# weleen/AGRL.pytorch

Hardware: AMD Instinct MI355X
Metric: frames/sec (fwd+GCN+distmat), MARS seq_len=8 (higher is better)
Workload: dtype fp16; 1 GPU; MARS seq_len=8 bs=32/GPU fp16 fwd+distmat (BASELINE configs[1]): 256x128 frames, VMGN ResNet50x2-branch + 2 graph layers, cosine distmat vs resident 12180 x 4096 gallery; global_batch=32, seq_len=8, gallery_rows_per_gpu=12180, parallelism=dp1, hip_graph=False, ranks=1, devices_visible=1, library=libagrl_hip.so, clip_batches_rotated=3, clip_bytes_rotated=301989888

## Files before the change

### agrl.pytorch_amd/csrc/agrl_common.h

```cpp
#pragma once
#include <hip/hip_runtime.h>
#include <math.h>
#include <stdint.h>
#include <stdio.h>
#include <stdarg.h>

#include "../../include/agrl_hip.h"

#define AGRL_WAVE 64

#ifndef AGRL_LP_F16
#define AGRL_LP_F16 1
#endif
constexpr bool kLpF16 = AGRL_LP_F16 != 0;
typedef unsigned short lp16_t;
typedef __attribute__((ext_vector_type(8))) __bf16 bf16x8_t;
typedef __attribute__((ext_vector_type(8))) _Float16 f16x8_t;
typedef __attribute__((ext_vector_type(4))) float f32x4_t;

void agrl_set_error(const char* fmt, ...);

#define AGRL_CHECK_ARG(cond, ...)       \
    do {                                \
        if (!(cond)) {                  \
            agrl_set_error(__VA_ARGS__); \
            return 1;                   \
        }                               \
    } while (0)

#define AGRL_CHECK_LAUNCH(name)                                                   \
    do {                                                                          \
        hipError_t e__ = hipGetLastError();                                       \
        if (e__ != hipSuccess) {                                                  \
            agrl_set_error("%s: launch failed: %s", name, hipGetErrorString(e__)); \
            return 2;                                                             \
        }                                                                         \
    } while (0)

static inline bool agrl_is_pow2(float v) {
    int e = 0;
    return v > 0.f && v <= 3.4e38f && frexpf(v, &e) == 0.5f;
}
#define AGRL_CHECK_POW2(value, who, name) \
    AGRL_CHECK_ARG(agrl_is_pow2(value), "%s: %s=%g is not a positive finite power of two", who, name, (double)(value))

__attribute__((visibility("hidden"))) int agrl_cu_count();

typedef __attribute__((address_space(3))) void lds_void_t;
typedef __attribute__((address_space(1))) const void gbl_void_t;

__host__ __device__ inline float lp16_to_f32(lp16_t v) {
    if constexpr (kLpF16) {
        return (float)__builtin_bit_cast(_Float16, v);
    } else {
        return __builtin_bit_cast(float, ((uint32_t)v) << 16);
    }
}

__host__ __device__ inline lp16_t f32_to_lp16(float f) {
    if constexpr (kLpF16) {
        return __builtin_bit_cast(unsigned short, (_Float16)f);
    } else {
#if defined(__HIP_DEVICE_COMPILE__)
        const __bf16 h = (__bf16)f;
        return __builtin_bit_cast(unsigned short, h);
#else
        uint32_t u = __builtin_bit_cast(uint32_t, f);
        if ((u & 0x7fffffffu) > 0x7f800000u) return (lp16_t)((u >> 16) | 0x40);
        u += 0x7fffu + ((u >> 16) & 1u);
        return (lp16_t)(u >> 16);
#endif
    }
}

__device__ inline uint32_t pack_lp16x2(float lo, float hi) {
    if constexpr (kLpF16) {
        typedef __attribute__((ext_vector_type(2))) _Float16 f16x2_t;
        const f16x2_t v = {(_Float16)lo, (_Float16)hi};
        return __builtin_bit_cast(uint32_t, v);
    } else {
        typedef __attribute__((ext_vector_type(2))) __bf16 bf16x2_t;
        const bf16x2_t v = {(__bf16)lo, (__bf16)hi};
        return __builtin_bit_cast(uint32_t, v);
    }
}

__device__ inline uint32_t pack_bf16x2(float lo, float hi) {
    typedef __attribute__((ext_vector_type(2))) __bf16 bf16x2_t;
    const bf16x2_t v = {(__bf16)lo, (__bf16)hi};
    return __builtin_bit_cast(uint32_t, v);
}

__device__ inline void unpack_lp16x2(uint32_t w, float& lo, float& hi) {
    if constexpr (kLpF16) {
        typedef __attribute__((ext_vector_type(2))) _Float16 f16x2_t;
        const f16x2_t v = __builtin_bit_cast(f16x2_t, w);
        lo = (float)v[0];
        hi = (float)v[1];
    } else {
        lo = __uint_as_float(w << 16);
        hi = __uint_as_float(w & 0xffff0000u);
    }
}

template <typename TA, typename TB>
__device__ inline __attribute__((ext_vector_type(4))) float mfma_lp16_16x16x32(const TA& a, const TB& b, __attribute__((ext_vector_type(4))) float c) {
    static_assert(sizeof(TA) == 16 && sizeof(TB) == 16, "16-byte MFMA operands");
    if constexpr (kLpF16) {
        return __builtin_amdgcn_mfma_f32_16x16x32_f16(__builtin_bit_cast(f16x8_t, a), __builtin_bit_cast(f16x8_t, b), c, 0, 0, 0);
    } else {
        return __builtin_amdgcn_mfma_f32_16x16x32_bf16(__builtin_bit_cast(bf16x8_t, a), __builtin_bit_cast(bf16x8_t, b), c, 0, 0, 0);
    }
}

__device__ inline float relu_nan(float v) { return __builtin_elementwise_maximum(v, 0.f); }

__device__ inline float wave_sum(float v) {
#pragma unroll
    for (int off = 32; off > 0; off >>= 1) v += __shfl_xor(v, off, 64);
    return v;
}

__device__ inline float wave_max(float v) {
#pragma unroll
    for (int off = 32; off > 0; off >>= 1) v = fmaxf(v, __shfl_xor(v, off, 64));
    return v;
}

__device__ inline int wave_sum_i(int v) {
#pragma unroll
    for (int off = 32; off > 0; off >>= 1) v += __shfl_xor(v, off, 64);
    return v;
}

template <typename T>
struct DT;
template <>
struct DT<float> {
    static constexpr int code = AGRL_F32;
    static constexpr int epc = 4;
    __device__ static inline float ld(const float* p) { return *p; }
    __device__ static inline void st(float* p, float v) { *p = v; }
};
struct f32s_t {
    float v;
};
template <>
struct DT<f32s_t> {
    static constexpr int code = AGRL_F32X3;
    static constexpr int epc = 4;
};
struct f32h_t {
    float v;
};
template <>
struct DT<f32h_t> {
    static constexpr int code = AGRL_F32H3;
    static constexpr int epc = 4;
};
template <>
struct DT<lp16_t> {
    static constexpr int code = AGRL_LP16;
    static constexpr int epc = 8;
    __device__ static inline float ld(const lp16_t* p) { return lp16_to_f32(*p); }
    __device__ static inline void st(lp16_t* p, float v) { *p = f32_to_lp16(v); }
};

static inline int cdiv(int a, int b) { return (a + b - 1) / b; }

#define AGRL_OPT_UNSET (-2147483647 - 1)
struct AgrlOpts {
    int igemm_wide;
    int pool_persist;
    int conv3x3_wide, conv3x3_c64;
    int distmat_tiled;
    int topk_radix;
    int graph_linear_mmajor;
    int conv3x3_n128;
    int conv3x3_fat_pb;
    int conv3x3_half, conv3x3_half_stagger;
    int stem_split_lds;
    int stem_xcd_map;
    int stem_regpool;
    int distmat_tile_n;
    int split16_ns;
    int duo_persist;
    int igemm_dbg, conv3x3_dbg;
};
const AgrlOpts& agrl_opts();
inline bool agrl_opt_set(int v) { return v != AGRL_OPT_UNSET; }

#ifdef AGRL_ABLATE
#define AGRL_DBG_BITS(p) ((p).dbg)
#else
#define AGRL_DBG_BITS(p) 0
#endif
```

### agrl.pytorch_amd/csrc/bottleneck_seam.hip

```cpp
#include <utility>

#include "igemm_dev.h"

namespace {

struct SeamParams {
    const unsigned char* y2;
    const unsigned char* wpk;
    const float* b3;
    const unsigned char* res;
    unsigned char* out;
    const float* b1n;
    unsigned char* z;
    int M;
};

#ifndef SEAM_ABL
#define SEAM_ABL 0
#endif
constexpr int SBM = 128;
constexpr int SCH = 256;

template <typename F, int... Is>
__device__ __forceinline__ void static_for_impl(F&& f, std::integer_sequence<int, Is...>) {
    (f(std::integral_constant<int, Is>{}), ...);
}
template <int N, typename F>
__device__ __forceinline__ void static_for(F&& f) {
    static_for_impl(f, std::make_integer_sequence<int, N>{});
}

typedef unsigned u32x4_t __attribute__((ext_vector_type(4)));
typedef __attribute__((address_space(3))) unsigned char lds_u8_t;
typedef __attribute__((address_space(3))) u32x4_t lds_u32x4_t;
__device__ __forceinline__ u32x4_t lds_ld16(const lds_u8_t* p) {
#if SEAM_ABL & 16
    return u32x4_t{(unsigned)(size_t)p, 1u, 2u, 3u};
#else
    return *reinterpret_cast<const lds_u32x4_t*>(p);
#endif
}

template <int IMM>
__device__ __forceinline__ void gload16_asm(u32x4_t& dst, unsigned off, const unsigned char* base) {
    static_assert(IMM >= 0 && IMM < 4096, "13-bit signed immediate");
    asm volatile("global_load_dwordx4 %0, %1, %2 offset:%3" : "=v"(dst) : "v"(off), "s"(base), "n"(IMM) : "memory");
}
template <int RQ>
__device__ __forceinline__ void mfma_v(f32x4_t& acc, const u32x4_t& b) {
    if constexpr (kLpF16) asm volatile("v_mfma_f32_16x16x32_f16 %0, a[%c2:%c3], %1, %0" : "+v"(acc) : "v"(b), "n"(4 * RQ), "n"(4 * RQ + 3));
    else asm volatile("v_mfma_f32_16x16x32_bf16 %0, a[%c2:%c3], %1, %0" : "+v"(acc) : "v"(b), "n"(4 * RQ), "n"(4 * RQ + 3));
}
template <int AQ, int RQ>
__device__ __forceinline__ void mfma_a(const u32x4_t& b) {
    if constexpr (kLpF16)
        asm volatile("v_mfma_f32_16x16x32_f16 a[%c1:%c2], a[%c3:%c4], %0, a[%c1:%c2]" ::"v"(b), "n"(4 * AQ), "n"(4 * AQ + 3), "n"(4 * RQ), "n"(4 * RQ + 3));
    else
        asm volatile("v_mfma_f32_16x16x32_bf16 a[%c1:%c2], a[%c3:%c4], %0, a[%c1:%c2]" ::"v"(b), "n"(4 * AQ), "n"(4 * AQ + 3), "n"(4 * RQ), "n"(4 * RQ + 3));
}
template <int AQ>
__device__ __forceinline__ void acc_zero() {
    asm volatile("v_accvgpr_write_b32 a[%c0], 0\n\tv_accvgpr_write_b32 a[%c1], 0\n\tv_accvgpr_write_b32 a[%c2], 0\n\tv_accvgpr_write_b32 a[%c3], 0" ::"n"(4 * AQ),
                 "n"(4 * AQ + 1), "n"(4 * AQ + 2), "n"(4 * AQ + 3));
}
template <int AQ>
__device__ __forceinline__ f32x4_t acc_read() {
    float x, y, z, w;
    asm volatile("v_accvgpr_read_b32 %0, a[%c4]\n\tv_accvgpr_read_b32 %1, a[%c5]\n\tv_accvgpr_read_b32 %2, a[%c6]\n\tv_accvgpr_read_b32 %3, a[%c7]"
                 : "=v"(x), "=v"(y), "=v"(z), "=v"(w)
                 : "n"(4 * AQ), "n"(4 * AQ + 1), "n"(4 * AQ + 2), "n"(4 * AQ + 3));
    return f32x4_t{x, y, z, w};
}
template <int IMM>
__device__ __forceinline__ void gstore16_asm(const u32x4_t& v, unsigned off, unsigned char* base) {
    asm volatile("global_store_dwordx4 %0, %1, %2 offset:%3\n\ts_nop 1" ::"v"(off), "v"(v), "s"(base), "n"(IMM) : "memory");
}
template <int RQ, int IMM>
__device__ __forceinline__ void ring_load(unsigned off, const unsigned char* base) {
    static_assert(IMM >= 0 && IMM < 4096, "13-bit signed immediate");
    asm volatile("global_load_dwordx4 a[%c2:%c3], %0, %1 offset:%4" ::"v"(off), "s"(base), "n"(4 * RQ), "n"(4 * RQ + 3), "n"(IMM) : "memory");
}
__device__ __forceinline__ void mfma_drain() { asm volatile("s_nop 15\n\ts_nop 15" ::: "memory"); }

__device__ __forceinline__ void dma16s(const unsigned char* sbase, unsigned voff, unsigned lds_wave_addr) {
    unsigned keep;
    asm volatile(
        "s_mov_b32 %0, m0\n\ts_mov_b32 m0, %3\n\ts_nop 0\n\tglobal_load_lds_dwordx4 %1, %2\n\ts_mov_b32 m0, %0"
        : "=&s"(keep)
        : "v"(voff), "s"(sbase), "s"(lds_wave_addr)
        : "memory");
}

constexpr int NWV = 4;
constexpr int FW1 = 4;
constexpr int Y2P = 4;
constexpr int S_OPS = (SEAM_ABL & 1) ? 0 : 32;
template <int KS1, int FW2, bool Y2RING, int RING>
struct Sched {
    static constexpr int G1F = FW1 * KS1, G2F = 8 * FW2, FPC = G1F + G2F;
    int allowed[FPC];
};
template <int KS1, int FW2, bool Y2RING, int RING>
constexpr Sched<KS1, FW2, Y2RING, RING> make_sched() {
    using S = Sched<KS1, FW2, Y2RING, RING>;
    S s{};
    int issued[4][S::FPC] = {};
    int seq = 0;
    for (int p = 0; p < RING; ++p) issued[0][p] = seq++;
    for (int k = 0; k < 3; ++k) {
        for (int p = 0; p < S::FPC; ++p) {
            if (p == S::G1F) seq += S_OPS;
            if (k == 1) s.allowed[p] = seq - 1 - issued[k][p];
            if (Y2RING && p < S::G1F && (p % FW1) == FW1 - 1 && ((p / FW1) & 1)) seq += Y2P;
            const int q = p + RING;
            if (q >= S::FPC) issued[k + 1][q - S::FPC] = seq++;
            else issued[k][q] = seq++;
        }
    }
    return s;
}
template <int KS1, int FW2, bool Y2RING, int RING>
struct SchedOf {
    static constexpr Sched<KS1, FW2, Y2RING, RING> value = make_sched<KS1, FW2, Y2RING, RING>();
};

template <int K1, int N1, int N2>
__global__ __launch_bounds__(NWV * 64) void bottleneck_seam_kernel(const SeamParams p) {
    static_assert((K1 == 256 || K1 == 512) && N1 % SCH == 0 && (N2 == 256 || N2 == 512), "shapes");
    constexpr int NC = N1 / SCH;
    constexpr int KS1 = K1 / 32;
    constexpr int FW2 = N2 / 64;
    constexpr bool Y2RING = K1 > 256;
    constexpr int NKT = K1 / 64;
    constexpr int NSL = 5, AHEAD = 3;
    constexpr int XO = Y2RING ? NSL * 16384 : 64 * 1024;
    constexpr int BIAS_OFF = XO + 64 * 1024;
    constexpr int RING = N2 == 256 ? 16 : 8;
    constexpr int NA2 = (64 - RING) < FW2 * 8 ? (64 - RING) : FW2 * 8;
    constexpr int NV2 = FW2 * 8 - NA2;
    using SCHED = SchedOf<KS1, FW2, Y2RING, RING>;
    constexpr int G1F = FW1 * KS1, G2F = 8 * FW2, FPC = G1F + G2F;
    static_assert(FPC % RING == 0, "the ring index of a fragment must not depend on the chunk");

    __shared__ __attribute__((aligned(16))) unsigned char smem_[BIAS_OFF + N1 * 4];
    lds_u8_t* const smem = (lds_u8_t*)smem_;
    const unsigned lds0 = (unsigned)(size_t)smem;

    const int tid = threadIdx.x;
    const int lane = tid & 63;
    const int wave = __builtin_amdgcn_readfirstlane(tid >> 6);
    const int frow = lane & 15, fchunk = lane >> 4;
    const int m0 = blockIdx.x * SBM;
    const unsigned lane16 = (unsigned)lane * 16u;

    unsigned a_off[2];
#pragma unroll
    for (int j = 0; j < 2; ++j) {
        const int row = wave * 32 + j * 8 + (lane >> 3);
        a_off[j] = (unsigned)(m0 + row) * (K1 * 2) + (unsigned)(((lane & 7) ^ ((row >> 1) & 7)) << 4);
    }
    const unsigned ldsA = __builtin_amdgcn_readfirstlane(lds0 + wave * 4096);
    auto issue_y2 = [&](int kt, int slot) {
        const unsigned char* src = p.y2 + kt * 128;
        const unsigned dst = ldsA + slot * 16384;
        dma16s(src, a_off[0], dst);
        dma16s(src, a_off[1], dst + 1024);
        dma16s(src + 16 * (K1 * 2), a_off[0], dst + 2048);
        dma16s(src + 16 * (K1 * 2), a_off[1], dst + 3072);
    };
    const int lo128 = frow * 128 + ((fchunk ^ ((frow >> 1) & 7)) << 4);
    const unsigned r_off = (unsigned)(m0 + frow) * (N1 * 2) + (unsigned)(wave * 64 + 8 * fchunk) * 2;

    const lds_u8_t* xptr = smem + XO + lane16;
    const lds_u8_t* sa0 = smem + lo128;
    const lds_u8_t* sa1 = smem + (lo128 ^ 64);
    asm volatile("" : "+v"(xptr), "+v"(sa0), "+v"(sa1));

    auto issue_w = [&](auto slot_c, const unsigned char* chunk_base, auto pos_c) {
        constexpr int SLOT = decltype(slot_c)::value, POS = decltype(pos_c)::value;
        if constexpr (SEAM_ABL & 8) return;
        ring_load<SLOT, (POS & 3) * 1024>(lane16, chunk_base + (POS & ~3) * 1024);
    };
    auto chunk_stream = [&](int c) { return p.wpk + (size_t)(c * NWV + wave) * (FPC * 1024); };

    f32x4_t acc1[FW1][8];
    asm volatile("" ::: "a255");
    static_for<NA2>([&](auto qc) { acc_zero<RING + decltype(qc)::value>(); });
    f32x4_t acc2v[NV2 > 0 ? NV2 : 1];
#pragma unroll
    for (int i = 0; i < (NV2 > 0 ? NV2 : 1); ++i) acc2v[i] = f32x4_t{0.f, 0.f, 0.f, 0.f};

    u32x4_t rres[8][2];
    auto load_residual = [&](int c) {
        const unsigned char* rc = p.res + (size_t)c * (SCH * 2);
#pragma unroll
        for (int b = 0; b < 8; ++b) {
            if constexpr (SEAM_ABL & 1) { rres[b][0] = u32x4_t{(unsigned)c, r_off, 1u, 2u}; rres[b][1] = rres[b][0]; continue; }
            gload16_asm<0>(rres[b][0], r_off, rc + b * (16 * N1 * 2));
            gload16_asm<64>(rres[b][1], r_off, rc + b * (16 * N1 * 2));
        }
    };
    auto init_acc1 = [&](int c) {
#pragma unroll
        for (int j = 0; j < 2; ++j) {
            float bias[8];
            {
                const lds_u8_t* bs = smem + BIAS_OFF + (c * SCH + wave * 64 + 32 * j + 8 * fchunk) * 4;
                const u32x4_t b0 = *reinterpret_cast<const lds_u32x4_t*>(bs), b1 = *reinterpret_cast<const lds_u32x4_t*>(bs + 16);
#pragma unroll
                for (int e = 0; e < 4; ++e) { bias[e] = __uint_as_float(b0[e]); bias[4 + e] = __uint_as_float(b1[e]); }
            }
#pragma unroll
            for (int b = 0; b < 8; ++b) {
                const uint32_t w4[4] = {rres[b][j][0], rres[b][j][1], rres[b][j][2], rres[b][j][3]};
                float v[8];
#pragma unroll
                for (int e = 0; e < 4; ++e) unpack_lp16x2(w4[e], v[2 * e], v[2 * e + 1]);
#pragma unroll
                for (int e = 0; e < 8; ++e) v[e] = (SEAM_ABL & 1) ? bias[e] : v[e] + bias[e];
                acc1[2 * j][b] = f32x4_t{v[0], v[1], v[2], v[3]};
                acc1[2 * j + 1][b] = f32x4_t{v[4], v[5], v[6], v[7]};
                __builtin_amdgcn_sched_barrier(0);
            }
        }
    };

    using std::integral_constant;

    load_residual(0);
#pragma unroll
    for (int i = 0; i < N1 / 1024; ++i)
        dma16s(reinterpret_cast<const unsigned char*>(p.b3) + (wave * (N1 / 1024) + i) * 1024, lane16, lds0 + BIAS_OFF + (wave * (N1 / 1024) + i) * 1024);
#pragma unroll
    for (int t = 0; t < (Y2RING ? AHEAD : NKT); ++t) issue_y2(t, t);
    {
        const unsigned char* s0 = chunk_stream(0);
        static_for<RING>([&](auto ic) { issue_w(ic, s0, ic); });
    }
    asm volatile("s_waitcnt vmcnt(%0)" ::"n"((SEAM_ABL & 8) ? 0 : RING) : "memory");
    __builtin_amdgcn_s_barrier();
    asm volatile("" ::: "memory");

    u32x4_t bf[8];
    int kt_slot = 0;
    int slot_off = 0;
    auto ld_y2 = [&](auto ks_c, int b) {
        constexpr int KS = decltype(ks_c)::value;
        const lds_u8_t* base = (KS & 1) ? sa1 : sa0;
        if constexpr (Y2RING) return lds_ld16(base + slot_off + b * 2048);
        else return lds_ld16(base + (KS >> 1) * 16384 + b * 2048);
    };

    for (int c = 0;; ++c) {
        const bool last = c + 1 == NC;
        const int cn = last ? 0 : c + 1;
        const unsigned char* ws = chunk_stream(c);
        const unsigned char* wsn = chunk_stream(cn);

#pragma unroll
        for (int b = 0; b < 8; ++b) asm volatile("" : "+v"(rres[b][0]), "+v"(rres[b][1]));
        init_acc1(c);
        __builtin_amdgcn_sched_barrier(0);
#pragma unroll
        for (int b = 0; b < 8; ++b) bf[b] = ld_y2(integral_constant<int, 0>{}, b);
        asm volatile("s_nop 4" ::: "memory");

        static_for<FPC>([&](auto pc) {
            constexpr int P = decltype(pc)::value;
            constexpr bool G1 = P < G1F;
            constexpr int F = G1 ? P : P - G1F;
            constexpr int FW = G1 ? FW1 : FW2;
            constexpr int KS = F / FW, A = F % FW;
            constexpr int SL = P % RING;
            constexpr bool LAST_A = A + 1 == FW;

            if constexpr (P == G1F) {
                if constexpr (!Y2RING) {
                    __builtin_amdgcn_s_barrier();
                    asm volatile("" ::: "memory");
                }
                mfma_drain();
                unsigned char* oc = p.out + (size_t)c * (SCH * 2);
                const lds_u8_t* xw = xptr + wave * 16384;
                static_for<2>([&](auto jc) {
                    constexpr int j = decltype(jc)::value;
#pragma unroll
                    for (int b = 0; b < 8; ++b) {
                        float v[8];
#pragma unroll
                        for (int e = 0; e < 4; ++e) {
                            v[e] = relu_nan(acc1[2 * j][b][e]);
                            v[4 + e] = relu_nan(acc1[2 * j + 1][b][e]);
                        }
                        const u32x4_t pk = {pack_lp16x2(v[0], v[1]), pack_lp16x2(v[2], v[3]), pack_lp16x2(v[4], v[5]), pack_lp16x2(v[6], v[7])};
                        if constexpr (!(SEAM_ABL & 1)) gstore16_asm<j * 64>(pk, r_off, oc + b * (16 * N1 * 2));
                        *reinterpret_cast<lds_u32x4_t*>(const_cast<lds_u8_t*>(xw) + (j * 8 + b) * 1024) = pk;
                    }
                });
                load_residual(cn);
                wg_barrier();
#pragma unroll
                for (int b = 0; b < 8; ++b) bf[b] = lds_ld16(xptr + b * 1024);
            }

            if constexpr (!(SEAM_ABL & 8)) wait_vmcnt<SCHED::value.allowed[P]>();

            if constexpr (Y2RING && G1 && LAST_A && (KS & 1)) {
                __builtin_amdgcn_s_barrier();
                asm volatile("" ::: "memory");
                const int nslot = (kt_slot + (KS >> 1) + 1) % NSL;
                issue_y2(((KS >> 1) + AHEAD) % NKT, (nslot + AHEAD - 1) % NSL);
                slot_off = nslot * 16384;
            }
            static_for<8>([&](auto bc) {
                constexpr int b = decltype(bc)::value;
                if constexpr (G1) {
                    if constexpr (SEAM_ABL & 2) asm volatile("" ::"v"(bf[b]));
                    else mfma_v<SL>(acc1[A][b], bf[b]);
                } else {
                    if constexpr (SEAM_ABL & 4) asm volatile("" ::"v"(bf[b]));
                    else if constexpr (A * 8 + b < NA2) mfma_a<RING + A * 8 + b, SL>(bf[b]);
                    else mfma_v<SL>(acc2v[A * 8 + b - NA2], bf[b]);
                }
                if constexpr (LAST_A) {
                    if constexpr (G1 && KS + 1 < KS1) {
                        __builtin_amdgcn_sched_barrier(0);
                        bf[b] = ld_y2(integral_constant<int, KS + 1>{}, b);
                    } else if constexpr (!G1 && KS + 1 < 8) {
                        __builtin_amdgcn_sched_barrier(0);
                        bf[b] = lds_ld16(xptr + ((KS + 1) * 8 + b) * 1024);
                    }
                }
            });
            __builtin_amdgcn_sched_barrier(0);
            constexpr int Q = P + RING;
            if constexpr (Q >= FPC) issue_w(integral_constant<int, SL>{}, wsn, integral_constant<int, Q - FPC>{});
            else issue_w(integral_constant<int, SL>{}, ws, integral_constant<int, Q>{});
            if constexpr (Y2RING && P + 1 == G1F) kt_slot = (kt_slot + NKT) % NSL;
        });
        if (last) break;
    }
    asm volatile("s_waitcnt vmcnt(0)" ::: "memory");
    mfma_drain();

    unsigned lane_z;
    asm volatile("v_mbcnt_lo_u32_b32 %0, -1, 0\n\tv_mbcnt_hi_u32_b32 %0, -1, %0" : "=v"(lane_z));
    const int frow_z = lane_z & 15, fchunk_z = lane_z >> 4;
    lp16_t* __restrict__ zp = reinterpret_cast<lp16_t*>(p.z);
    const int cb2 = wave * (N2 / NWV) + 8 * fchunk_z;
    static_for<FW2 / 2>([&](auto jc) {
        constexpr int j = decltype(jc)::value;
        const float4 b0 = *reinterpret_cast<const float4*>(p.b1n + cb2 + 32 * j);
        const float4 b1 = *reinterpret_cast<const float4*>(p.b1n + cb2 + 32 * j + 4);
        static_for<8>([&](auto bc) {
            constexpr int b = decltype(bc)::value;
            const int gm = m0 + b * 16 + frow_z;
            f32x4_t lo, hi;
            if constexpr ((2 * j) * 8 + b < NA2) lo = acc_read<RING + (2 * j) * 8 + b>();
            else lo = acc2v[(2 * j) * 8 + b - NA2];
            if constexpr ((2 * j + 1) * 8 + b < NA2) hi = acc_read<RING + (2 * j + 1) * 8 + b>();
            else hi = acc2v[(2 * j + 1) * 8 + b - NA2];
            float v[8];
            v[0] = lo[0] + b0.x; v[1] = lo[1] + b0.y; v[2] = lo[2] + b0.z; v[3] = lo[3] + b0.w;
            v[4] = hi[0] + b1.x; v[5] = hi[1] + b1.y; v[6] = hi[2] + b1.z; v[7] = hi[3] + b1.w;
#pragma unroll
            for (int e = 0; e < 8; ++e) v[e] = relu_nan(v[e]);
            *reinterpret_cast<uint4*>(zp + (size_t)gm * N2 + cb2 + 32 * j) =
                make_uint4(pack_lp16x2(v[0], v[1]), pack_lp16x2(v[2], v[3]), pack_lp16x2(v[4], v[5]), pack_lp16x2(v[6], v[7]));
        });
    });
}

__global__ void seam_pack_kernel(const lp16_t* __restrict__ w3, const lp16_t* __restrict__ w1n, uint4* __restrict__ wpk, int K1, int N1, int N2) {
    const int KS1 = K1 / 32, FW2 = N2 / 64, G1F = FW1 * KS1, FPC = G1F + 8 * FW2;
    const long long total = (long long)(N1 / SCH) * NWV * FPC * 64;
    for (long long t = blockIdx.x * (long long)blockDim.x + threadIdx.x; t < total; t += (long long)gridDim.x * blockDim.x) {
        const int lane = (int)(t & 63);
        long long r = t >> 6;
        const int q = (int)(r % FPC);
        r /= FPC;
        const int w = (int)(r % NWV), c = (int)(r / NWV);
        const int i = lane & 15, f = lane >> 4;
        const lp16_t* src;
        if (q < G1F) {
            const int ks = q / FW1, a = q % FW1;
            const int ch = c * SCH + w * 64 + 32 * (a >> 1) + 8 * (i >> 2) + 4 * (a & 1) + (i & 3);
            src = w3 + (size_t)ch * K1 + ks * 32 + f * 8;
        } else {
            const int g = q - G1F, ks = g / FW2, a = g % FW2;
            const int och = w * (N2 / NWV) + 32 * (a >> 1) + 8 * (i >> 2) + 4 * (a & 1) + (i & 3);
            src = w1n + (size_t)och * N1 + c * SCH + ks * 32 + f * 8;
        }
        wpk[t] = *reinterpret_cast<const uint4*>(src);
    }
}

bool seam_shape_ok(int Cmid, int Cout, int Cnext) {
    return (Cmid == 256 && Cout == 1024 && Cnext == 256) || (Cmid == 512 && Cout == 2048 && Cnext == 512) ||
           (Cmid == 256 && Cout == 1024 && Cnext == 512);
}

}

extern "C" long long agrl_bottleneck_seam_packed_bytes(int Cmid, int Cout, int Cnext) {
    if (!seam_shape_ok(Cmid, Cout, Cnext)) return 0;
    return ((long long)Cout * Cmid + (long long)Cnext * Cout) * 2;
}

extern "C" int agrl_bottleneck_seam_pack(const void* w3, const void* w1_next, void* packed, int Cmid, int Cout, int Cnext,
                                         agrl_stream_t stream) {
    AGRL_CHECK_ARG(w3 && w1_next && packed, "agrl_bottleneck_seam_pack: null pointer");
    AGRL_CHECK_ARG(seam_shape_ok(Cmid, Cout, Cnext), "agrl_bottleneck_seam_pack: built for 256/1024/256, 256/1024/512 and 512/2048/512 channels, got %d/%d/%d",
                   Cmid, Cout, Cnext);
    AGRL_CHECK_ARG((((uintptr_t)w3 | (uintptr_t)w1_next | (uintptr_t)packed) & 15) == 0, "agrl_bottleneck_seam_pack: pointers must be 16-byte aligned");
    hipLaunchKernelGGL(seam_pack_kernel, dim3(512), dim3(256), 0, (hipStream_t)stream, reinterpret_cast<const lp16_t*>(w3),
                       reinterpret_cast<const lp16_t*>(w1_next), reinterpret_cast<uint4*>(packed), Cmid, Cout, Cnext);
    AGRL_CHECK_LAUNCH("agrl_bottleneck_seam_pack");
    return 0;
}

extern "C" int agrl_bottleneck_seam(const void* y2, const void* packed, const float* b3, const void* residual, void* out,
                                    const float* b1_next, void* z, int M, int Cmid, int Cout, int Cnext, agrl_stream_t stream) {
    AGRL_CHECK_ARG(y2 && packed && b3 && residual && out && b1_next && z, "agrl_bottleneck_seam: null pointer");
    AGRL_CHECK_ARG(seam_shape_ok(Cmid, Cout, Cnext), "agrl_bottleneck_seam: built for 256/1024/256, 256/1024/512 and 512/2048/512 channels, got %d/%d/%d",
                   Cmid, Cout, Cnext);
    AGRL_CHECK_ARG(M > 0 && M % SBM == 0, "agrl_bottleneck_seam: the pixel count must be a multiple of %d (whole 16 x 8 frames), got %d", SBM, M);
    AGRL_CHECK_ARG((size_t)M * Cout * 2 < (1ull << 32), "agrl_bottleneck_seam: maps beyond 4 GB are not addressed");
    const uintptr_t al = (uintptr_t)y2 | (uintptr_t)packed | (uintptr_t)b3 | (uintptr_t)residual | (uintptr_t)out | (uintptr_t)b1_next | (uintptr_t)z;
    AGRL_CHECK_ARG((al & 15) == 0, "agrl_bottleneck_seam: pointers must be 16-byte aligned");
    SeamParams p;
    p.y2 = reinterpret_cast<const unsigned char*>(y2);
    p.wpk = reinterpret_cast<const unsigned char*>(packed);
    p.b3 = b3;
    p.res = reinterpret_cast<const unsigned char*>(residual);
    p.out = reinterpret_cast<unsigned char*>(out);
    p.b1n = b1_next;
    p.z = reinterpret_cast<unsigned char*>(z);
    p.M = M;
    const dim3 grid(M / SBM), block(NWV * 64);
    if (Cmid == 256 && Cnext == 256) hipLaunchKernelGGL((bottleneck_seam_kernel<256, 1024, 256>), grid, block, 0, (hipStream_t)stream, p);
    else if (Cmid == 256) hipLaunchKernelGGL((bottleneck_seam_kernel<256, 1024, 512>), grid, block, 0, (hipStream_t)stream, p);
    else hipLaunchKernelGGL((bottleneck_seam_kernel<512, 2048, 512>), grid, block, 0, (hipStream_t)stream, p);
    AGRL_CHECK_LAUNCH("agrl_bottleneck_seam");
    return 0;
}
```

### agrl.pytorch_amd/csrc/common.hip

```cpp
#include "agrl_common.h"

static thread_local char g_err[512] = "";

void agrl_set_error(const char* fmt, ...) {
    va_list ap;
    va_start(ap, fmt);
    vsnprintf(g_err, sizeof(g_err), fmt, ap);
    va_end(ap);
}

extern "C" int agrl_version(void) { return 100; }
extern "C" const char* agrl_last_error(void) { return g_err; }

extern "C" int agrl_lp16_is_f16(void) { return kLpF16 ? 1 : 0; }

#include <atomic>

int agrl_cu_count() {
    constexpr int kMaxDev = 64;
    static std::atomic<int> cache[kMaxDev];
    int dev = 0;
    if (hipGetDevice(&dev) != hipSuccess) return 256;
    const bool slot = dev >= 0 && dev < kMaxDev;
    int n = slot ? cache[dev].load(std::memory_order_relaxed) : 0;
    if (n > 0) return n;
    if (hipDeviceGetAttribute(&n, hipDeviceAttributeMultiprocessorCount, dev) != hipSuccess || n <= 0) n = 256;
    if (slot) cache[dev].store(n, std::memory_order_relaxed);
    return n;
}

#include <stdlib.h>

static int opt_int(const char* name) {
    const char* e = getenv(name);
    return e ? atoi(e) : AGRL_OPT_UNSET;
}
static int opt_flag(const char* name) {
    const char* e = getenv(name);
    return e && !(e[0] == '0' && e[1] == 0) ? 1 : 0;
}
static AgrlOpts load_opts() {
    AgrlOpts o;
    o.igemm_wide = opt_int("AGRL_IGEMM_WIDE");
    o.pool_persist = opt_flag("AGRL_POOL_PERSIST");
    o.conv3x3_wide = opt_int("AGRL_CONV3X3_WIDE");
    o.conv3x3_c64 = opt_int("AGRL_CONV3X3_C64");
    o.distmat_tiled = opt_flag("AGRL_DISTMAT_TILED");
    o.topk_radix = opt_flag("AGRL_TOPK_RADIX");
    o.graph_linear_mmajor = opt_flag("AGRL_GRAPH_LINEAR_MMAJOR");
    o.conv3x3_n128 = opt_flag("AGRL_CONV3X3_N128");
    o.distmat_tile_n = opt_int("AGRL_DISTMAT_TILE_N");
    o.duo_persist = opt_int("AGRL_DUO_PERSIST");
    o.split16_ns = opt_int("AGRL_SPLIT16_NS");
    o.stem_xcd_map = opt_int("AGRL_STEM_XCD_MAP");
    o.stem_split_lds = opt_int("AGRL_STEM_SPLIT_LDS");
    o.stem_regpool = opt_int("AGRL_STEM_REGPOOL");
    o.conv3x3_fat_pb = opt_int("AGRL_CONV3X3_FAT_PB");
    o.conv3x3_half = opt_int("AGRL_CONV3X3_HALF");
    o.conv3x3_half_stagger = opt_int("AGRL_CONV3X3_HALF_STAGGER");
#ifdef AGRL_ABLATE
    o.igemm_dbg = agrl_opt_set(opt_int("AGRL_IGEMM_DBG")) ? opt_int("AGRL_IGEMM_DBG") : 0;
    o.conv3x3_dbg = agrl_opt_set(opt_int("AGRL_CONV3X3_DBG")) ? opt_int("AGRL_CONV3X3_DBG") : 0;
#else
    o.igemm_dbg = 0;
    o.conv3x3_dbg = 0;
#endif
    return o;
}
static AgrlOpts g_opts = load_opts();

const AgrlOpts& agrl_opts() { return g_opts; }
extern "C" int agrl_reload_options(void) {
    g_opts = load_opts();
    return 0;
}
extern "C" int agrl_built_with_ablation(void) {
#ifdef AGRL_ABLATE
    return 1;
#else
    return 0;
#endif
}
```

### agrl.pytorch_amd/torchreid/_hip.py

```python
from __future__ import annotations

import ctypes as C
import os
import threading

import torch

F32 = 0
LP16 = 1
F32X3 = 2
F32H3P = 4
F32H3 = 3
FRAMES_NCHW = 0
FRAMES_NHWC = 1
METRIC_EUCLIDEAN = 0
METRIC_COSINE = 1

LP_NAME = os.environ.get("AGRL_HIP_LP16")
if LP_NAME is None:
    LP_NAME = os.environ.get("AGRL_HIP_PRECISION") if os.environ.get("AGRL_HIP_PRECISION") in ("fp16", "bf16") else "fp16"
if LP_NAME not in ("fp16", "bf16"):
    raise ValueError("AGRL_HIP_LP16 must be fp16 or bf16, not %r" % LP_NAME)
LP_DTYPE = torch.float16 if LP_NAME == "fp16" else torch.bfloat16

_HERE = os.path.dirname(os.path.abspath(__file__))
LIB_PATH = os.environ.get(
    "AGRL_HIP_LIB", os.path.normpath(os.path.join(_HERE, "..", "lib", "libagrl_hip.so" if LP_NAME == "fp16" else "libagrl_hip_bf16.so"))
)


class HipLibraryError(RuntimeError):
    """libagrl_hip.so is missing or incomplete."""


class HipKernelError(RuntimeError):
    """An entry point of libagrl_hip.so returned a non-zero status."""


_p = C.c_void_p
_i = C.c_int
_f = C.c_float

SIGNATURES = {
    "agrl_stem_conv_bn_relu_maxpool": [_p, _p, _p, _p, _i, _i, _i, _i, _p],
    "agrl_stem_conv_bn_relu_maxpool_lp16": [_p, _p, _p, _p, _i, _i, _i, _p],
    "agrl_conv2d_bn_act": [_p, _p, _p, _p, _p, _i, _i, _i, _i, _i, _i, _i, _i, _i, _i, _i, _p],
    "agrl_conv1x1_dual_split16": [_p, _p, _p, _p, _p] + [_i] * 8 + [_f, _i, _i, _p],
    "agrl_stem_split16": [_p, _p, _p, _p, _p, _i, _i, _i, _f, _p],
    "agrl_stem_conv_bn_relu_maxpool_u8": [_p, _p, _i, _p, _p, _p, _i, _i, _i, _i, _p],
    "agrl_stem_conv_bn_relu_maxpool_lp16_u8": [_p, _p, _i, _p, _p, _p, _i, _i, _i, _p],
    "agrl_stem_split16_u8": [_p, _p, _i, _p, _p, _p, _p, _i, _i, _i, _f, _p],
    "agrl_frames_normalize_u8": [_p, _p, _i, _p, _i, _i, _i, _p],
    "agrl_clip_resample_u8": [_p, _p, _p, _i, _i, _i, _i, _i, _p],
    "agrl_resample_taps_u8": [_i, _i, _p, _p, _p],
    "agrl_split16_planes": [_p, _p, C.c_longlong, _i, _i, _p],
    "agrl_split16_weight_planes": [_p, _p, C.c_longlong, _i, _f, _p],
    "agrl_split16_weights_inloop": [_p, _p, C.c_longlong, _i, _p],
    "agrl_conv1x1_split16": [_p, _p, _p, _p, _p, _i, _i, _i, _i, _f, _i, _p],
    "agrl_conv1x1_split16_dual": [_p, _p, _p, _p, _p, _i, _i, _i, _i, _i, _f, _i, _p],
    "agrl_conv1x1_split16_pool": [_p, _p, _p, _p, _p, _i, _i, _i, _i, _i, _i, C.POINTER(_i), _i, _i, _f, _i, _p],
    "agrl_conv3x3_packed_split16": [_p, _p, _p, _p, _i, _i, _i, _i, _i, _i, _f, _p],
    "agrl_conv2d_bn_act_split16": [_p, _p, _p, _p, _p] + [_i] * 10 + [_f, _i, _i, _p],
    "agrl_bottleneck_tail": [_p, _p, _p, _p, _p, _p, _p, _p, _p, _p, _p, _i, _i, _i, _i, _i, _p],
    "agrl_bottleneck_seam_packed_bytes": [_i, _i, _i],
    "agrl_bottleneck_seam_pack": [_p, _p, _p, _i, _i, _i, _p],
    "agrl_bottleneck_seam": [_p, _p, _p, _p, _p, _p, _p, _i, _i, _i, _i, _p],
    "agrl_conv3x3_packed_bytes": [_i, _i],
    "agrl_conv1x1_packed_bytes": [_i, _i],
    "agrl_conv1x1_pack": [_p, _p, _i, _i, _p],
    "agrl_conv1x1_packed_bn_act": [_p, _p, _p, _p, _p, _i, _i, _i, _i, _i, _p],
    "agrl_conv1x1_packed_res_bn_act": [_p, _p, _p, _p, _p, _i, _i, _i, _i, _p],
    "agrl_conv1x1_packed_res_pool": [_p, _p, _p, _p, _p, _p, _i, _i, _i, _i, _i, _i, C.POINTER(_i), _i, _i, _p],
    "agrl_conv1x1_packed_dual_duo": [_p, _p, _p, _p, _p, _i, _i, _i, _i, _i, _p],
    "agrl_conv1x1_packed_dual_strided": [_p, _p, _p, _p, _p, _i, _i, _i, _i, _i, _i, _i, _i, _p],
    "agrl_conv3x3_pack": [_p, _p, _i, _i, _p],
    "agrl_conv3x3_packed_bn_act": [_p, _p, _p, _p, _i, _i, _i, _i, _i, _i, _p],
    "agrl_bottleneck_block": [_p, _p, _p, _p, _p, _p, _p, _p, _p, _p, _p, _p, _p, _i, _i, _i, _i, _i, _i, _p],
    "agrl_conv1x1_dual_bn_act": [_p, _p, _p, _p, _p, _i, _i, _i, _i, _i, _p],
    "agrl_conv1x1_bn_act_pool": [_p, _p, _p, _p, _p, _p, _p, _i, _i, _i, _i, _i, _i, C.POINTER(_i), _i, _i, _p],
    "agrl_linear_nobias": [_p, _p, _p, _i, _i, _i, _i, _p],
    "agrl_part_pool": [_p, _p, _p, _p, _p, _i, _i, _i, _i, C.POINTER(_i), _i, _i, _p],
    "agrl_clip_pool": [_p, _p, _i, _i, _i, _i, _p],
    "agrl_clip_pool_ragged": [_p, _p, _p, _p, _i, _i, _i, _i, _p],
    "agrl_graph_gram": [_p, _p, _i, _i, _i, _i, _p],
    "agrl_graph_pair_product": [_p, _p, _p, _p, _i, _i, _i, _p],
    "agrl_graph_finalize": [_p, _i, _p, _p, _i, _i, _i, _i, _i, _p],
    "agrl_graph_propagate": [_p, _p, _p, _p, _p, _f, _f, _f, _p, _p, _i, _i, _i, _p],
    "agrl_pam_pool": [_p, _p, _p, _p, _i, _i, _i, _i, _i, C.POINTER(_i), _i, _i, _p],
    "agrl_pam_combine": [_p, _p, _p, _f, _p, _p, _i, _i, _p],
    "agrl_pam_pool_train": [_p, _p, _p, _p, _p, _i, _i, _i, _i, _i, C.POINTER(_i), _i, _i, _p],
    "agrl_pam_pool_backward": [_p, _p, _p, _p, _p, _p, _p, _i, _i, _i, _i, _i, C.POINTER(_i), _i, _i, _p],
    "agrl_pam_combine_train": [_p, _p, _p, _p, _p, _i, _i, _p],
    "agrl_pam_combine_backward": [_p, _p, _p, _p, _p, _p, _p, _p, _i, _i, _p, C.c_size_t, _p],
    "agrl_col_sum_workspace": [_i, _i],
    "agrl_col_sum": [_p, _p, _i, _i, _p, C.c_size_t, _p],
    "agrl_graph_apply": [_p, _p, _p, _i, _i, _i, _i, _p],
    "agrl_graph_tracklet_operand": [_p, _p, _i, _p, _p, _i, _i, _i, _i, _i, _i, _i, _p],
    "agrl_graph_finalize_bits": [_p, _i, _p, _p, _i, _i, _i, _i, _i, _p],
    "agrl_pose_adjacency_bits": [_p, _p, _p, _i, _i, _i, _i, C.c_float, C.c_float, _p],
    "agrl_adjacency_pack": [_p, _p, _i, _i, _p],
    "agrl_graph_linear_mix": [_p, _p, _p, _p, _p, _f, _f, _f, _p, _i, _i, _i, _i, _p],
    "agrl_row_sqnorm": [_p, _p, _i, _i, _i, _p],
    "agrl_attn_pool_bnneck": [_p, _p, _p, _p, _p, _p, _p, _p, _p, _p, _i, _i, _i, _i, _i, _p],
    "agrl_sta_frame_stats": [_p, _p, _p, _p, _i, _i, _i, _i, _i, _p],
    "agrl_sta_fuse": [_p, _p, _p, _p, _p, _p, _i, _i, _i, _i, _i, _i, _p],
    "agrl_linear_bn_relu": [_p, _p, _p, _p, _p, _i, _i, _i, _i, _p],
    "agrl_attn_tail": [_p, _p, _p, _p, _p, _p, _p, _p, _p, _p, _p, _p, _p, _i, _i, _i, _i, _i, _p],
    "agrl_row_l2_normalize": [_p, _p, _i, _i, _i, _i, _i, _p],
    "agrl_distmat_split16": [_p, _p, _p, _p, _p, _i, _i, _i, _i, _i, _f, _p, C.c_size_t, _p],
    "agrl_distmat": [_p, _p, _p, _p, _p, _i, _i, _i, _i, _i, _i, _p, C.c_size_t, _p],
    "agrl_pose_adjacency": [_p, _p, _p, _i, _i, _i, _i, C.c_float, C.c_float, _p],
    "agrl_re_ranking_workspace": [_i, _i, _i],
    "agrl_re_ranking": [_p, _p, _p, _i, _i, _i, _i, C.c_double, _p, _i, _p, C.c_size_t, _p],
    "agrl_rank_topk": [_p, _i, _i, _i, _i, _i, _p, _p, _p],
    "agrl_distmat_topk_workspace": [_i, _i],
    "agrl_distmat_topk": [_p, _p, _p, _p, _i, _i, _i, _i, _i, _i, _i, _p, _p, _p, C.c_size_t, _p, C.c_size_t, _p],
    "agrl_rank_argsort": [_p, _i, _i, _i, _p, _p],
    "agrl_rank_mars": [_p, _p, _p, _p, _p, _i, _i, _i, _p, _p, _p],
    "agrl_rank_market1501": [_p, _i, _i, _i, _p, _p, _p, _p, _i, _p, _p, _p, _p],
    "agrl_triplet_hard_mine": [_p, _p, _i, _i, _p, _p, _p, _p, _p],
    "agrl_axpby": [_p, _p, _f, _f, _p, C.c_size_t, _p],
    "agrl_part_pool_backward": [_p, _p, _p, _p, _i, _i, _i, _i, _i, C.POINTER(_i), _i, _p],
    "agrl_attn_pool_backward": [_p, _p, _p, _i, _i, _i, _i, _p],
    "agrl_graph_matrix_backward": [_p, _i, _p, _p, _i, _i, _i, _i, _p],
    "agrl_xent_label_smooth": [_p, _p, _i, _i, _f, _p, _p, _p, _p],
    "agrl_triplet_loss": [_p, _p, _i, _i, _f, _i, _p, _p, _p, _p, _p, _p, _p, _p],
    "agrl_bn_workspace": [_i, _i],
    "agrl_bn_stats": [_p, _p, _p, _i, _i, _p, C.c_size_t, _p],
    "agrl_conv2d_stats": [_p, _p, _p, _p, C.c_size_t] + [_i] * 10 + [_p],
    "agrl_bn_stats_from_partials": [_p, _i, _i, _i, _p, _p, _p, C.c_size_t, _p],
    "agrl_bn_fold_train": [_p, _p, _p, _p, _f, _f, C.c_longlong, _p, _p, _p, _p, _p, _p, _i, _p],
    "agrl_bn_apply": [_p, _p, _p, _p, _p, _p, _i, _i, _i, _f, _p],
    "agrl_bn_backward": [_p, _p, _p, _p, _p, _p, _p, _i, _f, _p, _p, _p, _p, _i, _i, _p, C.c_size_t, _p],
    "agrl_im2col_t": [_p, _p, _i, _i, _i, _i, _i, _i, _i, _i, _i, _p],
    "agrl_gemm_nt_splitk": [_p, _p, _p, _i, _i, _i, _i, _p, C.c_size_t, _p],
    "agrl_im2col_rows": [_p, _p] + [_i] * 10 + [_p],
    "agrl_conv_wgrad_workspace": [_i] * 9,
    "agrl_conv_wgrad_plan": [_i] * 10 + [C.POINTER(_i)],
    "agrl_conv_wgrad": [_p, _p, _p] + [_i] * 10 + [_p, C.c_size_t, _p],
    "agrl_maxpool3x3s2": [_p, _p, _p, _i, _i, _i, _i, _p],
    "agrl_maxpool3x3s2_backward": [_p, _p, _p, _i, _i, _i, _i, _p],
    "agrl_diag_read_stream": [_p, C.c_size_t, _p, _i, _p],
    "agrl_optim_geometry": [C.POINTER(_i), C.POINTER(_i), C.POINTER(_i)],
    "agrl_adam_step": [_p, _i, _p, _i] + [_f] * 7 + [_i, _i, _p],
    "agrl_sgd_step": [_p, _i, _p, _i, _f, _f, _f, _i, _i, _i, _i, _p],
    "agrl_rmsprop_step": [_p, _i, _p, _i] + [_f] * 6 + [_i, _i, _p],
    "agrl_adabound_step": [_p, _i, _p, _i] + [_f] * 8 + [_i, _i, _p],
    "agrl_radam_step": [_p, _i, _p, _i] + [_f] * 6 + [_i, _i, _p],
}

_lock = threading.Lock()
_lib = None


def lib():
    global _lib
    if _lib is not None:
        return _lib
    with _lock:
        if _lib is not None:
            return _lib
        if not os.path.exists(LIB_PATH):
            raise HipLibraryError(
                "libagrl_hip.so not found at %s -- build it with `python __graft_entry__.py` "
                "(or `make -C agrl.pytorch_amd/csrc`); the HIP path has no fallback" % LIB_PATH
            )
        try:
            h = C.CDLL(LIB_PATH)
        except OSError as e:
            raise HipLibraryError("cannot load %s: %s" % (LIB_PATH, e))
        for name, argtypes in SIGNATURES.items():
            try:
                fn = getattr(h, name)
            except AttributeError:
                raise HipLibraryError("%s does not export %s" % (LIB_PATH, name))
            fn.argtypes = argtypes
            fn.restype = _i
        h.agrl_re_ranking_workspace.restype = C.c_size_t
        h.agrl_bn_workspace.restype = C.c_size_t
        h.agrl_col_sum_workspace.restype = C.c_size_t
        h.agrl_conv_wgrad_workspace.restype = C.c_size_t
        h.agrl_distmat_topk_workspace.restype = C.c_size_t
        h.agrl_bottleneck_seam_packed_bytes.restype = C.c_longlong
        h.agrl_conv3x3_packed_bytes.restype = C.c_longlong
        h.agrl_conv1x1_packed_bytes.restype = C.c_longlong
        for name in ("agrl_reload_options", "agrl_built_with_ablation", "agrl_lp16_is_f16"):
            getattr(h, name).argtypes = []
            getattr(h, name).restype = _i
        h.agrl_version.restype = _i
        h.agrl_last_error.restype = C.c_char_p
        if bool(h.agrl_lp16_is_f16()) != (LP_NAME == "fp16"):
            raise HipLibraryError("%s stores 16-bit data as %s but AGRL_HIP_LP16 asks for %s" % (
                LIB_PATH, "fp16" if h.agrl_lp16_is_f16() else "bf16", LP_NAME))
        _lib = h
    return _lib


RELOAD_HOOKS = []


def reload_options():
    lib().agrl_reload_options()
    for hook in RELOAD_HOOKS:
        hook()


def available() -> bool:
    try:
        lib()
        return True
    except HipLibraryError:
        return False


def _check(name, status):
    if status != 0:
        msg = lib().agrl_last_error()
        raise HipKernelError("%s failed (%d): %s" % (name, status, msg.decode() if msg else "?"))


def stream_ptr(device=None):
    return torch.cuda.current_stream(device).cuda_stream


def ptr(t):
    if t is None:
        return None
    assert t.is_cuda, "HIP entry points take device tensors"
    assert t.is_contiguous(), "HIP entry points take contiguous tensors"
    return t.data_ptr()


def dtype_code(dt):
    if dt == torch.float32:
        return F32
    if dt == LP_DTYPE:
        return LP16
    raise TypeError("unsupported dtype %s (float32 / %s only: the loaded library's 16-bit type is %s)" % (dt, LP_DTYPE, LP_NAME))


PROFILE = None
PROFILE_TAG = None


def call(name, *args):
    fn = getattr(lib(), name)
    if PROFILE is None:
        _check(name, fn(*args))
        return
    stream = torch.cuda.ExternalStream(args[-1]) if args[-1] else torch.cuda.current_stream()
    start, end = torch.cuda.Event(enable_timing=True), torch.cuda.Event(enable_timing=True)
    start.record(stream)
    _check(name, fn(*args))
    end.record(stream)
    global PROFILE_TAG
    PROFILE.append((name, start, end, PROFILE_TAG))
    PROFILE_TAG = None
```

### agrl.pytorch_amd/torchreid/hip_ops.py

```python
from __future__ import annotations

import ctypes as C
import functools
import os

import numpy as np
import torch

from . import _hip
from ._hip import F32, LP16, LP_DTYPE, LP_NAME, METRIC_COSINE, METRIC_EUCLIDEAN, call, dtype_code, ptr


import contextlib
import threading
import weakref

_MODE = threading.local()


@contextlib.contextmanager
def f32_split(on=True):
    prev = getattr(_MODE, 'split', False)
    _MODE.split = bool(on)
    try:
# ... 312 lines not shown
                 _stream(x_nchw))
    return out


def conv_bn_act(x, w_ohwi, bias, stride, pad, relu, residual=None, x_presplit=False, out_presplit=False):
    N, H, W, Cin = x.shape
    Cout, R, S, Cin2 = w_ohwi.shape
    assert Cin == Cin2 and x.dtype == w_ohwi.dtype
    OH, OW = (H + 2 * pad - R) // stride + 1, (W + 2 * pad - S) // stride + 1
    out = torch.empty((N, OH, OW, Cout), dtype=x.dtype, device=x.device)
    if residual is not None:
        assert residual.shape == out.shape and residual.dtype == out.dtype
    if _hip.PROFILE is not None:
        e = x.element_size()
        _hip.PROFILE_TAG = {"flops": 2.0 * N * OH * OW * Cout * R * S * Cin,
                            "bytes": e * (x.numel() + w_ohwi.numel() + out.numel() * (2 if residual is not None else 1)),
                            "conv": (R, stride, Cin, Cout, OH, OW)}
    unscale = getattr(w_ohwi, 'agrl_unscale', None)
    with _dev(x):
        if unscale is not None:
            assert x.dtype == torch.float32 and getattr(w_ohwi, 'agrl_presplit', False), "fp16x3 weights come from split16_inloop_weights"
            call("agrl_conv2d_bn_act_split16", ptr(x), ptr(w_ohwi), ptr(bias), ptr(residual), ptr(out), N, H, W, Cin, Cout, R, S,
                 stride, pad, 1 if relu else 0, float(unscale), 1 if x_presplit else 0, 1 if out_presplit else 0, _stream(x))
        else:
            assert not (x_presplit or out_presplit), "pre-split activations exist in the 'fp16x3' arithmetic only"
            call("agrl_conv2d_bn_act", ptr(x), ptr(w_ohwi), ptr(bias), ptr(residual), ptr(out), N, H, W, Cin, Cout, R, S,
                 stride, pad, 1 if relu else 0, _gemm_code(x.dtype), _stream(x))
    return out


def conv1x1_dual_split16(x, x2, w_cat, bias, stride, relu=True, x2_presplit=False, out_planes=0):
    N, H, W, K1 = x.shape
    K2 = x2.shape[3]
    Cout = w_cat.shape[0]
    OH, OW = (H - 1) // stride + 1, (W - 1) // stride + 1
    assert x.dtype == torch.float32 and x2.dtype == torch.float32 and x.is_contiguous() and x2.is_contiguous()
    assert tuple(x2.shape[:3]) == (N, OH, OW) and tuple(w_cat.shape) == (Cout, K1 + K2) and getattr(w_cat, 'agrl_presplit', False)
    assert out_planes in (0, 2, 3)
    out = (torch.empty((N, OH, OW, out_planes * Cout), dtype=torch.float16, device=x.device) if out_planes
           else torch.empty((N, OH, OW, Cout), dtype=torch.float32, device=x.device))
    if _hip.PROFILE is not None:
        M = N * OH * OW
        _hip.PROFILE_TAG = {"flops": 2.0 * M * Cout * (K1 + K2), "bytes": 4.0 * (M * (K1 + K2) + w_cat.numel()) + out.numel() * out.element_size(),
                            "conv": (1, stride, K1 + K2, Cout, OH, OW)}
    with _dev(x):
        call("agrl_conv1x1_dual_split16", ptr(x), ptr(x2), ptr(w_cat), ptr(bias), ptr(out), N, H, W, stride, K1, K2, Cout,
             1 if relu else 0, float(w_cat.agrl_unscale), 1 if x2_presplit else 0, int(out_planes), _stream(x))
    return out


def split16_prescale(w):
    import math
    amax = float(w.detach().abs().max())
    if not (amax > 0.0 and math.isfinite(amax)):
        k = 0
    else:
        k = 13 - math.frexp(amax)[1] + 1
    ws = (w.detach().float() * (2.0 ** k)).contiguous()
    ws.agrl_unscale = 2.0 ** (-k)
    return ws


def split16_inloop_weights(w):
    ws = split16_prescale(w)
    K = ws.shape[-1]
    assert K % 32 == 0, "the in-loop split needs whole 32-element k-tiles (K = %d)" % K
    t = ws.view(-1, K // 32, 2, 4, 4).permute(0, 1, 3, 2, 4)
    hi = t.to(torch.float16)
    lo = (t - hi.float()).to(torch.float16)
    out = torch.stack([hi, lo], dim=2).contiguous().view(torch.float32).view(ws.shape)
    out.agrl_unscale = ws.agrl_unscale
    out.agrl_presplit = True
    out.agrl_scaled = ws
    return out


def split16_true_weights(t):
    src = t.agrl_scaled if getattr(t, 'agrl_presplit', False) else t
    return src * t.agrl_unscale


def pack_stem_weights_split16(w_ohwi):
    assert tuple(w_ohwi.shape) == (64, 7, 7, 3)
    ws = split16_prescale(w_ohwi)
    w4 = torch.zeros((64, 7, 8, 4), dtype=torch.float32, device=w_ohwi.device)
    w4[:, :, :7, :3] = ws
    wh = w4.to(torch.float16)
    wl = (w4 - wh.float()).to(torch.float16)
    out = []
    for t in (wh, wl):
        packed = torch.zeros((64, 240), dtype=torch.float16, device=w_ohwi.device)
        packed[:, :224] = t.view(64, 224)
        out.append(packed.contiguous())
    return out[0], out[1], ws.agrl_unscale


def stem_split16(x_nchw, wh_packed, wl_packed, unscale, bias, mean=PIXEL_MEAN, std=PIXEL_STD):
    x_nchw, N, H, W, ebytes, u8 = _stem_frames(x_nchw, mean, std)
    CH, CW, PH, PW = stem_out_shape(H, W)
    out = torch.empty((N, PH, PW, 64), dtype=torch.float32, device=x_nchw.device)
    if _hip.PROFILE is not None:
        _hip.PROFILE_TAG = {"flops": 2.0 * N * CH * CW * 64 * 147, "bytes": ebytes * x_nchw.numel() + 4.0 * out.numel() + 4.0 * wh_packed.numel(),
                            "conv": (7, 2, 3, 64, PH, PW)}
    with _dev(x_nchw):
        if u8 is not None:
            call("agrl_stem_split16_u8", ptr(x_nchw), ptr(u8[0]), u8[1], ptr(wh_packed), ptr(wl_packed), ptr(bias), ptr(out), N, H, W,
                 float(unscale), _stream(x_nchw))
        else:
            call("agrl_stem_split16", ptr(x_nchw), ptr(wh_packed), ptr(wl_packed), ptr(bias), ptr(out), N, H, W, float(unscale), _stream(x_nchw))
    return out


def split16_planes_available():
    return LP_NAME == 'fp16'


def split16_plane_weights(w, segments=None, pair_first=False):
    ws = split16_prescale(w)
    parts = []
    for i, seg in enumerate(torch.split(ws, segments or [ws.shape[-1]], dim=-1)):
        wh = seg.to(torch.float16)
        wl = (seg - wh.float()).to(torch.float16)
        wh_s = (wh.float() * (2.0 ** -11)).to(torch.float16)
        if pair_first and i == 0:
            assert seg.shape[-1] % 128 == 0
            lead = tuple(seg.shape[:-1])
            slabs = [t.reshape(lead + (-1, 128)) for t in (wh, wl, wh_s)]
            parts.append(torch.stack(slabs, dim=-2).reshape(lead + (3 * seg.shape[-1],)))
        else:
            parts += [wh, wh_s, wl]
    return torch.cat(parts, dim=-1).contiguous(), ws.agrl_unscale


def to_split16_planes(x, nplanes=3):
    assert x.dtype == torch.float32 and x.is_contiguous() and x.shape[-1] % 4 == 0 and nplanes in (2, 3)
    Cc = x.shape[-1]
    out = torch.empty(tuple(x.shape[:-1]) + (nplanes * Cc,), dtype=torch.float16, device=x.device)
    with _dev(x):
        call("agrl_split16_planes", ptr(x), ptr(out), x.numel() // Cc, Cc, nplanes, _stream(x))
    return out


def to_split16_weight_planes(x, scale):
    assert x.dtype == torch.float32 and x.is_contiguous() and x.dim() == 2 and x.shape[1] % 4 == 0
    out = torch.empty((x.shape[0], 3 * x.shape[1]), dtype=torch.float16, device=x.device)
    with _dev(x):
        call("agrl_split16_weight_planes", ptr(x), ptr(out), x.shape[0], x.shape[1], float(scale), _stream(x))
    return out


def distmat_split16(q3, g3, metric, g_unscale, qn=None, gn=None, out=None):
    m, D3 = q3.shape
    n = g3.shape[0]
    assert g3.shape[1] == D3 and q3.dtype == torch.float16 and g3.dtype == torch.float16
    if out is None:
        out = torch.empty((m, n), dtype=torch.float32, device=q3.device)
    code = METRIC_EUCLIDEAN if metric == "euclidean" else METRIC_COSINE
    if _hip.PROFILE is not None:
        _hip.PROFILE_TAG = {"flops": 2.0 * m * n * D3 / 3, "mfma_flops": 2.0 * m * n * D3, "bytes": 2.0 * (m + n) * D3 + 4.0 * m * n}
    ws = None
    if (-(-m // 64)) * (-(-n // 128)) < 256:
        ws = torch.empty((8 * m * n,), dtype=torch.float32, device=q3.device)
    with _dev(q3):
        call("agrl_distmat_split16", ptr(q3), ptr(g3), ptr(qn), ptr(gn), out.data_ptr(), m, n, D3, out.stride(0), code, float(g_unscale),
             ptr(ws), 0 if ws is None else ws.numel() * 4, _stream(q3))
    return out


def from_split16_planes(x3, nplanes=3):
    Cc = x3.shape[-1] // nplanes
    return x3[..., :Cc].float() + x3[..., Cc:2 * Cc].float() * (2.0 ** -11)


def conv1x1_split16(x3, packed, unscale, bias, Cout, residual3=None, relu=True, x2=None, layout=0):
    N, H, W, Kx = x3.shape
    K3 = Kx // 2 * 3 if layout & 1 else Kx
    K23 = 0 if x2 is None else x2.shape[3]
    M = N * H * W
    no = 2 if layout & 2 else 3
    assert x3.dtype == torch.float16 and x3.is_contiguous() and packed.numel() == 2 * (K3 + K23) * Cout
    assert residual3 is None or (residual3.dtype == torch.float16 and residual3.is_contiguous() and tuple(residual3.shape) == (N, H, W, no * Cout))
    out = torch.empty((N, H, W, no * Cout), dtype=torch.float16, device=x3.device)
    if _hip.PROFILE is not None:
        _hip.PROFILE_TAG = {"flops": 2.0 * M * Cout * (K3 + K23) / 3, "mfma_flops": 2.0 * M * Cout * (K3 + K23),
                            "bytes": 2.0 * (x3.numel() + (0 if x2 is None else x2.numel()) + out.numel() + (0 if residual3 is None else residual3.numel() * 2 // no)) + packed.numel()}
    with _dev(x3):
        if x2 is None:
            call("agrl_conv1x1_split16", ptr(x3), ptr(packed), ptr(bias), ptr(residual3), ptr(out), M, K3, Cout, 1 if relu else 0,
                 float(unscale), int(layout), _stream(x3))
        else:
            assert residual3 is None and x2.dtype == torch.float16 and x2.is_contiguous() and tuple(x2.shape[:3]) == (N, H, W)
            call("agrl_conv1x1_split16_dual", ptr(x3), ptr(x2), ptr(packed), ptr(bias), ptr(out), M, K3, K23, Cout, 1 if relu else 0,
                 float(unscale), int(layout), _stream(x3))
    return out


def conv1x1_split16_pool(x3, packed, unscale, bias, Cout, residual3, splits, mean, relu=True, layout=0):
    N, H, W, K3 = x3.shape
    assert x3.dtype == torch.float16 and x3.is_contiguous() and (H, W) == (16, 8) and packed.numel() == 2 * K3 * Cout
    assert not (layout & 1), "the pooled conv's input is conv2's output: a triple"
    assert residual3 is None or (residual3.dtype == torch.float16 and residual3.is_contiguous()
                                 and tuple(residual3.shape) == (N, H, W, (2 if layout & 2 else 3) * Cout))
    P = int(sum(splits))
    pooled = torch.empty((N, P, Cout), dtype=torch.float32, device=x3.device)
    arr = (C.c_int * len(splits))(*[int(s_) for s_ in splits])
    if _hip.PROFILE is not None:
        _hip.PROFILE_TAG = {"flops": 2.0 * N * H * W * Cout * K3 / 3, "mfma_flops": 2.0 * N * H * W * Cout * K3,
                            "bytes": 2.0 * (x3.numel() + (residual3.numel() if residual3 is not None else 0)) + packed.numel() + 4.0 * pooled.numel()}
    with _dev(x3):
        call("agrl_conv1x1_split16_pool", ptr(x3), ptr(packed), ptr(bias), ptr(residual3), ptr(pooled), N, H, W, K3, Cout,
             1 if relu else 0, arr, len(splits), 1 if mean else 0, float(unscale), int(layout), _stream(x3))
    return pooled


def conv3x3_split16(x3, packed, unscale, bias, Cout, relu=True):
    N, H, W, Cin3 = x3.shape
    assert x3.dtype == torch.float16 and x3.is_contiguous() and packed.numel() == 2 * 9 * Cin3 * Cout
    out = torch.empty((N, H, W, 3 * Cout), dtype=torch.float16, device=x3.device)
    if _hip.PROFILE is not None:
        _hip.PROFILE_TAG = {"flops": 2.0 * N * H * W * Cout * 9 * Cin3 / 3, "mfma_flops": 2.0 * N * H * W * Cout * 9 * Cin3,
                            "bytes": 2.0 * (x3.numel() + out.numel()) + packed.numel()}
    with _dev(x3):
        call("agrl_conv3x3_packed_split16", ptr(x3), ptr(packed), ptr(bias), ptr(out), N, H, W, Cin3, Cout, 1 if relu else 0,
             float(unscale), _stream(x3))
    return out


def conv1x1_dual_supported(x1, x2, w_cat):
    K1, K2 = x1.shape[-1], x2.shape[-1]
    return (x1.dtype == LP_DTYPE and x2.dtype == LP_DTYPE and K1 == 2 * K2 and K1 % 64 == 0
            and w_cat.shape[0] % 256 == 0 and x1.shape[:-1] == x2.shape[:-1])


def conv1x1_dual(x1, x2, w_cat, bias, relu=True):
    N, H, W, K1 = x1.shape
    K2 = x2.shape[-1]
    Cout = w_cat.shape[0]
    assert tuple(w_cat.shape) == (Cout, K1 + K2) and w_cat.dtype == x1.dtype
    out = torch.empty((N, H, W, Cout), dtype=x1.dtype, device=x1.device)
    M = N * H * W
    if _hip.PROFILE is not None:
        _hip.PROFILE_TAG = {"flops": 2.0 * M * Cout * (K1 + K2), "bytes": 2.0 * (x1.numel() + x2.numel() + w_cat.numel() + out.numel()),
                            "conv": (1, 1, K1 + K2, Cout, H, W)}
    with _dev(x1):
        call("agrl_conv1x1_dual_bn_act", ptr(x1), ptr(x2), ptr(w_cat), ptr(bias), ptr(out), M, K1, K2, Cout, 1 if relu else 0,
             _stream(x1))
    return out


def conv1x1_bn_act_pool(x, w_ohwi, bias, residual, splits, mean, want_lp, relu=True):
    N, H, W, Cin = x.shape
    Cout = w_ohwi.shape[0]
    assert x.dtype == LP_DTYPE and tuple(w_ohwi.shape[1:3]) == (1, 1) and H * W == 128
    P = int(sum(splits))
    pooled = torch.empty((N, P, Cout), dtype=torch.float32, device=x.device)
    pooled_lp = torch.empty((N, P, Cout), dtype=LP_DTYPE, device=x.device) if want_lp else None
    arr = (C.c_int * len(splits))(*[int(s) for s in splits])
    if _hip.PROFILE is not None:
        _hip.PROFILE_TAG = {"flops": 2.0 * N * H * W * Cout * Cin,
                            "bytes": 2.0 * (x.numel() + w_ohwi.numel() + (residual.numel() if residual is not None else 0)) + 4.0 * pooled.numel()}
    with _dev(x):
        call("agrl_conv1x1_bn_act_pool", ptr(x), ptr(w_ohwi), ptr(bias), ptr(residual), None, ptr(pooled), ptr(pooled_lp),
             N, H, W, Cin, Cout, 1 if relu else 0, arr, len(splits), 1 if mean else 0, _stream(x))
    return pooled, pooled_lp


SEAM_SHAPES = ((256, 1024, 256), (512, 2048, 512), (256, 1024, 512))


def bottleneck_seam_supported(w3, w1_next, pixels=None):
    return (w3.dtype == LP_DTYPE and w1_next.dtype == LP_DTYPE and w3.dim() == 4 and tuple(w3.shape[1:3]) == (1, 1)
            and (w3.shape[3], w3.shape[0], w1_next.shape[0]) in SEAM_SHAPES and tuple(w1_next.shape[1:]) == (1, 1, w3.shape[0])
            and (pixels is None or pixels % 128 == 0))


def bottleneck_seam_pack(w3, w1_next):
    assert bottleneck_seam_supported(w3, w1_next)
    Cout, Cmid, Cnext = w3.shape[0], w3.shape[3], w1_next.shape[0]
    w3, w1_next = w3.contiguous(), w1_next.contiguous()
    nbytes = int(_hip.lib().agrl_bottleneck_seam_packed_bytes(Cmid, Cout, Cnext))
    assert nbytes == 2 * (w3.numel() + w1_next.numel())
    packed = torch.empty((nbytes,), dtype=torch.uint8, device=w3.device)
    with _dev(w3):
        call("agrl_bottleneck_seam_pack", ptr(w3), ptr(w1_next), ptr(packed), Cmid, Cout, Cnext, _stream(w3))
    return packed


def bottleneck_seam(y2, packed, b3, residual, b1_next, dims):
    Cmid, Cout, Cnext = dims
    N, H, W, C = y2.shape
    M = N * H * W
    assert y2.dtype == LP_DTYPE and C == Cmid and residual.shape == (N, H, W, Cout) and residual.dtype == y2.dtype and M % 128 == 0
    assert y2.is_contiguous() and residual.is_contiguous()
    out = torch.empty((N, H, W, Cout), dtype=y2.dtype, device=y2.device)
    z = torch.empty((N, H, W, Cnext), dtype=y2.dtype, device=y2.device)
    if _hip.PROFILE is not None:
        _hip.PROFILE_TAG = {"flops": 2.0 * M * (Cmid * Cout + Cout * Cnext),
                            "bytes": 2.0 * (y2.numel() + residual.numel() + out.numel() + z.numel()) + packed.numel(),
                            "conv": (1, 1, Cmid, Cout, H, W)}
    with _dev(y2):
        call("agrl_bottleneck_seam", ptr(y2), ptr(packed), ptr(b3), ptr(residual), ptr(out), ptr(b1_next), ptr(z), M, Cmid, Cout,
             Cnext, _stream(y2))
    return out, z


def conv3x3_packed_enabled():
    return True


def conv3x3_packed_supported(w_ohwi, H=None, W=None):
    return (w_ohwi.dtype == LP_DTYPE and w_ohwi.dim() == 4 and tuple(w_ohwi.shape[1:3]) == (3, 3) and w_ohwi.shape[3] % 64 == 0
            and w_ohwi.shape[3] >= 128 and (w_ohwi.shape[0] % 256 == 0 or w_ohwi.shape[0] == 128) and (H is None or (H % 16 == 0 and W % 8 == 0)))


def conv3x3_pack(w_ohwi):
    assert conv3x3_packed_supported(w_ohwi)
    Cout, Cin = w_ohwi.shape[0], w_ohwi.shape[3]
    if Cout == 128:
        w_ohwi = torch.cat([w_ohwi, torch.zeros_like(w_ohwi)], dim=0)
        Cout = 256
    w_ohwi = w_ohwi.contiguous()
    nbytes = int(_hip.lib().agrl_conv3x3_packed_bytes(Cin, Cout))
    assert nbytes == 2 * w_ohwi.numel()
    packed = torch.empty((nbytes,), dtype=torch.uint8, device=w_ohwi.device)
    with _dev(w_ohwi):
        call("agrl_conv3x3_pack", ptr(w_ohwi), ptr(packed), Cin, Cout, _stream(w_ohwi))
    return packed


def conv3x3_packed(x, packed, bias, Cout, relu=True):
    N, H, W, Cin = x.shape
    assert x.dtype == LP_DTYPE and x.is_contiguous() and packed.numel() == 2 * 9 * Cin * max(Cout, 256)
    out = torch.empty((N, H, W, Cout), dtype=x.dtype, device=x.device)
    if _hip.PROFILE is not None:
        _hip.PROFILE_TAG = {"flops": 2.0 * N * H * W * 9 * Cin * Cout, "bytes": 2.0 * (x.numel() + out.numel()) + 2.0 * 9 * Cin * Cout,
                            "conv": (3, 1, Cin, Cout, H, W)}
    with _dev(x):
        call("agrl_conv3x3_packed_bn_act", ptr(x), ptr(packed), ptr(bias), ptr(out), N, H, W, Cin, Cout, 1 if relu else 0, _stream(x))
    return out


def conv1x1_packed_supported(w):
    w2 = w.reshape(w.shape[0], -1) if w.dim() == 4 and tuple(w.shape[1:3]) == (1, 1) else w
    return w2.dtype == LP_DTYPE and w2.dim() == 2 and w2.shape[1] % 128 == 0 and w2.shape[0] % 256 == 0


def conv1x1_pack(w):
    assert conv1x1_packed_supported(w)
    w = w.reshape(w.shape[0], -1).contiguous()
    Cout, K = w.shape
    nbytes = int(_hip.lib().agrl_conv1x1_packed_bytes(K, Cout))
    assert nbytes == 2 * w.numel()
    packed = torch.empty((nbytes,), dtype=torch.uint8, device=w.device)
    with _dev(w):
        call("agrl_conv1x1_pack", ptr(w), ptr(packed), K, Cout, _stream(w))
    return packed


def conv1x1_packed(x, packed, bias, Cout, relu=True, x2=None, duo=False):
    N, H, W, K1 = x.shape
    K2 = 0 if x2 is None else x2.shape[3]
    M = N * H * W
    assert x.dtype == LP_DTYPE and x.is_contiguous() and packed.numel() == 2 * (K1 + K2) * Cout
    assert x2 is None or (x2.dtype == x.dtype and x2.is_contiguous() and tuple(x2.shape[:3]) == (N, H, W))
    out = torch.empty((N, H, W, Cout), dtype=x.dtype, device=x.device)
    if _hip.PROFILE is not None:
        _hip.PROFILE_TAG = {"flops": 2.0 * M * (K1 + K2) * Cout,
                            "bytes": 2.0 * (x.numel() + (0 if x2 is None else x2.numel()) + out.numel()) + packed.numel(),
                            "conv": (1, 1, K1 + K2, Cout, H, W)}
    with _dev(x):
        if duo and x2 is not None:
            call("agrl_conv1x1_packed_dual_duo", ptr(x), ptr(x2), ptr(packed), ptr(bias), ptr(out), M, K1, K2, Cout, 1 if relu else 0, _stream(x))
        else:
            call("agrl_conv1x1_packed_bn_act", ptr(x), ptr(x2), ptr(packed), ptr(bias), ptr(out), M, K1, K2, Cout, 1 if relu else 0, _stream(x))
    return out


def conv1x1_packed_dual_strided(x, x2, packed, bias, Cout, stride, relu=True):
    N, Hi, Wi, K1 = x.shape
    Ho, Wo = (Hi - 1) // stride + 1, (Wi - 1) // stride + 1
    K2 = x2.shape[3]
    assert x.dtype == LP_DTYPE and x2.dtype == LP_DTYPE and x.is_contiguous() and x2.is_contiguous()
    assert tuple(x2.shape[:3]) == (N, Ho, Wo) and packed.numel() == 2 * (K1 + K2) * Cout
    out = torch.empty((N, Ho, Wo, Cout), dtype=x.dtype, device=x.device)
    M = N * Ho * Wo
    if _hip.PROFILE is not None:
        _hip.PROFILE_TAG = {"flops": 2.0 * M * (K1 + K2) * Cout, "bytes": 2.0 * (M * K1 + x2.numel() + out.numel()) + packed.numel(),
                            "conv": (1, 1, K1 + K2, Cout, Ho, Wo)}
    with _dev(x):
        call("agrl_conv1x1_packed_dual_strided", ptr(x), ptr(x2), ptr(packed), ptr(bias), ptr(out), N, Hi, Wi, stride, K1, K2, Cout,
             1 if relu else 0, _stream(x))
    return out


def conv1x1_packed_res(x, packed, bias, Cout, residual, relu=True):
    N, H, W, K = x.shape
    M = N * H * W
    assert x.dtype == LP_DTYPE and x.is_contiguous() and packed.numel() == 2 * K * Cout
    assert residual is None or (residual.dtype == x.dtype and residual.is_contiguous() and tuple(residual.shape) == (N, H, W, Cout))
    out = torch.empty((N, H, W, Cout), dtype=x.dtype, device=x.device)
    if _hip.PROFILE is not None:
        _hip.PROFILE_TAG = {"flops": 2.0 * M * K * Cout,
                            "bytes": 2.0 * (x.numel() + out.numel() * (2 if residual is not None else 1)) + packed.numel(),
                            "conv": (1, 1, K, Cout, H, W)}
    with _dev(x):
        call("agrl_conv1x1_packed_res_bn_act", ptr(x), ptr(packed), ptr(bias), ptr(residual), ptr(out), M, K, Cout, 1 if relu else 0,
             _stream(x))
    return out


def conv1x1_packed_res_pool(x, packed, bias, Cout, residual, splits, mean, want_lp, relu=True):
    N, H, W, K = x.shape
    assert x.dtype == LP_DTYPE and x.is_contiguous() and (H, W) == (16, 8) and packed.numel() == 2 * K * Cout
    assert residual is None or (residual.dtype == x.dtype and residual.is_contiguous() and tuple(residual.shape) == (N, H, W, Cout))
    P = int(sum(splits))
    pooled = torch.empty((N, P, Cout), dtype=torch.float32, device=x.device)
    pooled_lp = torch.empty((N, P, Cout), dtype=LP_DTYPE, device=x.device) if want_lp else None
    arr = (C.c_int * len(splits))(*[int(s) for s in splits])
    if _hip.PROFILE is not None:
        _hip.PROFILE_TAG = {"flops": 2.0 * N * H * W * Cout * K,
                            "bytes": 2.0 * (x.numel() + (residual.numel() if residual is not None else 0)) + packed.numel() + 4.0 * pooled.numel()}
    with _dev(x):
        call("agrl_conv1x1_packed_res_pool", ptr(x), ptr(packed), ptr(bias), ptr(residual), ptr(pooled), ptr(pooled_lp),
             N, H, W, K, Cout, 1 if relu else 0, arr, len(splits), 1 if mean else 0, _stream(x))
    return pooled, pooled_lp


def bottleneck_tail_supported(y2, w3, w1_next, shortcut_conv=None):
    if (y2.dtype == LP_DTYPE and tuple(w3.shape) == (512, 1, 1, 128) and tuple(w1_next.shape) == (128, 1, 1, 512)
            and shortcut_conv is None):
        return True
    ok = (y2.dtype == LP_DTYPE and tuple(w3.shape) == (256, 1, 1, 64)
          and tuple(w1_next.shape) in ((64, 1, 1, 256), (128, 1, 1, 256)))
    if shortcut_conv is not None:
        ok = ok and tuple(shortcut_conv[0].shape) == (256, 1, 1, 64) and shortcut_conv[1] == 1 and w1_next.shape[0] == 64
    return ok


def bottleneck_tail(y2, w3, b3, residual, w1_next, b1_next, shortcut=None):
    N, H, W, Cmid = y2.shape
    Cout, Cnext = w3.shape[0], w1_next.shape[0]
    assert y2.dtype == LP_DTYPE and (residual is None) != (shortcut is None)
    xs = ws = bs = None
    Cshort = 0
    if shortcut is not None:
        xs, ws, bs = shortcut
        assert xs.shape[:3] == y2.shape[:3] and xs.dtype == y2.dtype
        Cshort = xs.shape[3]
    else:
        assert residual.shape == (N, H, W, Cout) and residual.dtype == y2.dtype
    out = torch.empty((N, H, W, Cout), dtype=y2.dtype, device=y2.device)
    z = torch.empty((N, H, W, Cnext), dtype=y2.dtype, device=y2.device)
    M = N * H * W
    if _hip.PROFILE is not None:
        rd = (residual.numel() if residual is not None else xs.numel() + ws.numel())
        _hip.PROFILE_TAG = {"flops": 2.0 * M * ((Cmid + Cshort) * Cout + Cout * Cnext),
                            "bytes": 2.0 * (y2.numel() + rd + out.numel() + z.numel() + w3.numel() + w1_next.numel())}
    with _dev(y2):
        call("agrl_bottleneck_tail", ptr(y2), ptr(w3), ptr(b3), ptr(residual), ptr(xs), ptr(ws), ptr(bs), ptr(out),
             ptr(w1_next), ptr(b1_next), ptr(z), M, Cmid, Cout, Cnext, Cshort, _stream(y2))
    return out, z


def bottleneck_block_supported(z, w2, stride, w3, w1_next, shortcut_conv=None):
    ok = (z.dtype == LP_DTYPE and stride == 1 and tuple(w2.shape) == (64, 3, 3, 64) and tuple(w3.shape) == (256, 1, 1, 64)
          and tuple(w1_next.shape) in ((64, 1, 1, 256), (128, 1, 1, 256)) and z.shape[1] % 8 == 0 and z.shape[2] % 8 == 0)
    if shortcut_conv is not None:
        ok = ok and tuple(shortcut_conv[0].shape) == (256, 1, 1, 64) and shortcut_conv[1] == 1 and w1_next.shape[0] == 64
    return ok


def bottleneck_block(z, w2, b2, w3, b3, residual, w1_next, b1_next, shortcut=None):
    N, H, W, Cmid = z.shape
    Cout, Cnext = w3.shape[0], w1_next.shape[0]
    assert z.dtype == LP_DTYPE and (residual is None) != (shortcut is None)
    xs = ws = bs = None
    if shortcut is not None:
        xs, ws, bs = shortcut
        assert tuple(xs.shape) == (N, H, W, 64) and xs.dtype == z.dtype
    else:
        assert tuple(residual.shape) == (N, H, W, Cout) and residual.dtype == z.dtype
    out = torch.empty((N, H, W, Cout), dtype=z.dtype, device=z.device)
    zn = torch.empty((N, H, W, Cnext), dtype=z.dtype, device=z.device)
    M = N * H * W
    if _hip.PROFILE is not None:
        rd = residual.numel() if residual is not None else xs.numel() + ws.numel()
        _hip.PROFILE_TAG = {"flops": 2.0 * M * (9 * Cmid * Cmid + (Cmid + (64 if shortcut is not None else 0)) * Cout + Cout * Cnext),
                            "bytes": 2.0 * (z.numel() + rd + out.numel() + zn.numel() + w2.numel() + w3.numel() + w1_next.numel())}
    with _dev(z):
        call("agrl_bottleneck_block", ptr(z), ptr(w2), ptr(b2), ptr(w3), ptr(b3), ptr(residual), ptr(xs), ptr(ws), ptr(bs),
             ptr(out), ptr(w1_next), ptr(b1_next), ptr(zn), N, H, W, Cmid, Cout, Cnext, _stream(z))
    return out, zn


def linear_nobias(x, w):
    M, K = x.shape
    Nout, K2 = w.shape
    assert K == K2 and x.dtype == w.dtype
    y = torch.empty((M, Nout), dtype=torch.float32, device=x.device)
    if _hip.PROFILE is not None:
        _hip.PROFILE_TAG = {"flops": 2.0 * M * K * Nout, "bytes": x.element_size() * (x.numel() + w.numel()) + 4 * y.numel()}
    with _dev(x):
        call("agrl_linear_nobias", ptr(x), ptr(w), ptr(y), M, K, Nout, _gemm_code(x.dtype), _stream(x))
    return y


def part_pool(x4_1, x4_2, splits, want_lp):
    F_, h, w, Cc = x4_1.shape
    assert x4_2.shape == x4_1.shape and x4_1.dtype == x4_2.dtype
    P = int(sum(splits))
    gsum = torch.empty((F_, Cc), dtype=torch.float32, device=x4_1.device)
    nodes = torch.empty((F_, P, Cc), dtype=torch.float32, device=x4_1.device)
    nodes_lp = torch.empty((F_, P, Cc), dtype=LP_DTYPE, device=x4_1.device) if want_lp else None
    arr = (C.c_int * len(splits))(*[int(s) for s in splits])
    with _dev(x4_1):
        call("agrl_part_pool", ptr(x4_1), ptr(x4_2), ptr(gsum), ptr(nodes), ptr(nodes_lp), F_, h, w, Cc, arr,
             len(splits), dtype_code(x4_1.dtype), _stream(x4_1))
    return gsum, nodes, nodes_lp


GRAM_CSLICE = 128


def graph_matrix(f, adj, use_pose, learn_graph, mask_diag=False):
    B, V, Cc = f.shape
    G = torch.empty((B, V, V), dtype=torch.float32, device=f.device)
    gram = None
    nz = 0
    with _dev(f):
        if learn_graph:
            nz = Cc // GRAM_CSLICE
            gram = torch.empty((B, nz, V, V), dtype=torch.float32, device=f.device)
            call("agrl_graph_gram", ptr(f), ptr(gram), B, V, Cc, GRAM_CSLICE, _stream(f))
        if use_pose and adjacency_is_packed(adj):
            assert tuple(adj.shape) == (B, V, (V + 31) // 32)
            call("agrl_graph_finalize_bits", ptr(gram), nz, ptr(adj.contiguous()), ptr(G), B, V, 1, 1 if learn_graph else 0,
                 1 if mask_diag else 0, _stream(f))
            return G
        if use_pose:
            assert adj is not None and tuple(adj.shape) == (B, V, V) and adj.dtype == torch.float32
            adj = adj.contiguous()
        call("agrl_graph_finalize", ptr(gram), nz, ptr(adj) if use_pose else None, ptr(G), B, V,
             1 if use_pose else 0, 1 if learn_graph else 0, 1 if mask_diag else 0, _stream(f))
    return G


def adjacency_is_packed(adj):
    return adj is not None and adj.dtype == torch.int32


def adjacency_pack(adj):
    B, V, V2 = adj.shape
    assert V == V2 and adj.dtype == torch.float32
    bits = torch.empty((B, V, (V + 31) // 32), dtype=torch.int32, device=adj.device)
    with _dev(adj):
        call("agrl_adjacency_pack", ptr(adj.contiguous()), ptr(bits), B, V, _stream(adj))
    return bits


def adjacency_pack_host(adj):
    import numpy as np
    a = np.asarray(adj.detach().cpu() if hasattr(adj, "detach") else adj) != 0
    B, V, _ = a.shape
    W = (V + 31) // 32
    pad = np.zeros((B, V, W * 32), dtype=bool)
    pad[:, :, :V] = a
    words = (pad.reshape(B, V, W, 32).astype(np.uint64) << np.arange(32, dtype=np.uint64)).sum(axis=3).astype(np.uint32)
    return torch.from_numpy(words.view(np.int32).copy())


def graph_propagate(f, h, G, bn_scale, bn_shift, gamma, slope, want_lp, keep=None):
    if keep is None:
        keep = 1.0 - float(gamma)
    B, V, Cc = f.shape
    out = torch.empty_like(f)
    out_lp = torch.empty((B, V, Cc), dtype=LP_DTYPE, device=f.device) if want_lp else None
    if _hip.PROFILE is not None:
        _hip.PROFILE_TAG = {"flops": 2.0 * B * V * V * Cc, "bytes": 4.0 * (3 * B * V * Cc + B * V * V)}
    with _dev(f):
        call("agrl_graph_propagate", ptr(f), ptr(h), ptr(G), ptr(bn_scale), ptr(bn_shift), float(keep), float(gamma),
             float(slope), ptr(out), ptr(out_lp), B, V, Cc, _stream(f))
    return out, out_lp


def graph_apply_presplit_supported(f):
    B, V, Cc = f.shape
    return V <= 64 and V % 4 == 0 and Cc % 128 == 0


def graph_apply_operand(G, f, out_dtype, presplit=False):
    B, V, Cc = f.shape
    assert f.dtype == torch.float32 and G.dtype == torch.float32 and tuple(G.shape) == (B, V, V)
    assert not presplit or (out_dtype == torch.float32 and graph_apply_presplit_supported(f))
    if V <= 64 and V % 4 == 0 and Cc % 128 == 0:
        out = torch.empty((B, V, Cc), dtype=out_dtype, device=f.device)
        if _hip.PROFILE is not None:
            _hip.PROFILE_TAG = {"flops": 2.0 * B * V * V * Cc, "bytes": 4.0 * (B * V * Cc + B * V * V) + out.element_size() * B * V * Cc}
        with _dev(f):
            call("agrl_graph_apply", ptr(G.contiguous()), ptr(f.contiguous()), ptr(out), _hip.F32H3P if presplit else dtype_code(out_dtype), B, V, Cc,
                 _stream(f))
        return out
    key = (f.device, Cc)
    if key not in _UNIT:
        _UNIT[key] = (torch.ones((Cc,), dtype=torch.float32, device=f.device), torch.zeros((Cc,), dtype=torch.float32, device=f.device))
    one, zero = _UNIT[key]
    out, out_lp = graph_propagate(f, f, G, one, zero, 1.0, 1.0, want_lp=out_dtype == LP_DTYPE, keep=0.0)
# ... 836 lines not shown
```

### agrl.pytorch_amd/torchreid/models/_resnet_hip.py

```python
from __future__ import annotations

import os

import torch

from torchreid import hip_ops as ops

PRECISIONS = {'fp32': torch.float32, ops.LP_NAME: ops.LP_DTYPE, 'bf16x3': torch.float32, 'fp16x3': torch.float32}


def init_hip_attributes(model, train=False, train_tail=False):
    model.hip_precision = os.environ.get('AGRL_HIP_PRECISION', 'fp32')
    ops.check_precision(model.hip_precision)
    model.hip_static_weights = False
    if train:
        model.hip_train = os.environ.get('AGRL_HIP_TRAIN', '1') != '0'
        model.hip_train_precision = os.environ.get('AGRL_HIP_TRAIN_PRECISION', 'fp32')
    if train_tail:
        model.hip_train_tail = os.environ.get('AGRL_HIP_TRAIN_TAIL', '1') != '0'
    model._hip_packs = {}
    model.pixel_mean = (0.485, 0.456, 0.406)
    model.pixel_std = (0.229, 0.224, 0.225)


def fold_conv_bn(conv, bn, dtype, split16=False):
    w = conv.weight.detach().float()
    scale = bn.weight.detach().float() / torch.sqrt(bn.running_var.detach().float() + bn.eps)
    shift = bn.bias.detach().float() - bn.running_mean.detach().float() * scale
    w = (w * scale.view(-1, 1, 1, 1)).permute(0, 2, 3, 1).contiguous()
    if split16:
        assert dtype == torch.float32
        return ops.split16_inloop_weights(w), shift.contiguous()
    return w.to(dtype).contiguous(), shift.contiguous()


def fold_bn1d(bn):
    scale = bn.weight.detach().float() / torch.sqrt(bn.running_var.detach().float() + bn.eps)
    shift = bn.bias.detach().float() - bn.running_mean.detach().float() * scale
    return scale.contiguous(), shift.contiguous()


def check_packed_range(pack, where="vmgn"):
    def walk(obj, path):
        if torch.is_tensor(obj):
            if obj.dtype == ops.LP_DTYPE and obj.numel() and not bool(torch.isfinite(obj).all()):
                raise FloatingPointError("%s: the BatchNorm-folded weights of %s overflow %s (abs-max of the fp32 fold is beyond its "
                                         "range): load the bf16 build (AGRL_HIP_LP16=bf16) or use hip_precision='fp32'" % (where, path, ops.LP_NAME))
        elif isinstance(obj, dict):
            for k, v in obj.items():
                walk(v, "%s.%s" % (path, k))
        elif isinstance(obj, (list, tuple)):
            for i, v in enumerate(obj):
                walk(v, "%s[%d]" % (path, i))
    walk({k: v for k, v in pack.items() if k != 'fingerprint'}, "pack")


def pack_tensors(obj):
    if torch.is_tensor(obj):
        yield obj
    elif isinstance(obj, (dict, list, tuple)):
        for v in (obj.values() if isinstance(obj, dict) else obj):
            yield from pack_tensors(v)


def dual_weights(blk, wd=None, w3=None):
    wd, w3 = blk['ds'][0] if wd is None else wd, blk['c3'][0] if w3 is None else w3
    cout = w3.shape[0]
    return torch.cat([wd.view(cout, -1), w3.view(cout, -1)], dim=1).contiguous(), (blk['ds'][1] + blk['c3'][1]).contiguous()


def pack_stage(stage, dtype, seam=False, split16=False):
    blocks = []
    for unit in stage:
        blk = {
            'c1': fold_conv_bn(unit.conv1, unit.bn1, dtype, split16),
            'c2': fold_conv_bn(unit.conv2, unit.bn2, dtype, split16),
            'c3': fold_conv_bn(unit.conv3, unit.bn3, dtype, split16),
            'stride': unit.conv2.stride[0],
            'ds': None,
        }
        if unit.downsample is not None:
            blk['ds'] = fold_conv_bn(unit.downsample[0], unit.downsample[1], dtype, split16)
            blk['ds_stride'] = unit.downsample[0].stride[0]
            if split16 and blk['ds_stride'] == blk['stride'] and blk['ds'][0].shape[3] % 32 == 0 and blk['c3'][0].shape[3] % 32 == 0:
                w, b = dual_weights(blk, ops.split16_true_weights(blk['ds'][0]), ops.split16_true_weights(blk['c3'][0]))
                blk['dual16'] = (ops.split16_inloop_weights(w), b)
            if dtype == ops.LP_DTYPE and blk['ds_stride'] == 1 and blk['stride'] == 1:
                blk['dual'] = dual_weights(blk)
                if (ops.conv1x1_packed_supported(blk['dual'][0]) and blk['dual'][0].shape[1] >= 1536
                        and blk['ds'][0].shape[3] % 128 == 0 and blk['c3'][0].shape[3] % 128 == 0):
                    blk['dualp'] = ops.conv1x1_pack(blk['dual'][0])
            if dtype == ops.LP_DTYPE and blk['ds_stride'] > 1 and blk['ds_stride'] == blk['stride']:
                dual_w, dual_b = dual_weights(blk)
                if (ops.conv1x1_packed_supported(dual_w) and blk['ds'][0].shape[3] % 128 == 0 and blk['c3'][0].shape[3] % 128 == 0):
                    blk['dualps'] = ops.conv1x1_pack(dual_w)
                    blk['dualps_bias'] = dual_b
        if dtype == ops.LP_DTYPE and ops.conv1x1_packed_supported(blk['c1'][0]) and blk['c1'][0].shape[3] >= 1024:
            blk['c1p'] = ops.conv1x1_pack(blk['c1'][0])
        if (dtype == ops.LP_DTYPE and blk['ds'] is None and ops.conv1x1_packed_supported(blk['c3'][0])
                and blk['c3'][0].shape[0] >= 2048):
            blk['c3p'] = ops.conv1x1_pack(blk['c3'][0])
        if dtype == ops.LP_DTYPE and blk['stride'] == 1 and ops.conv3x3_packed_supported(blk['c2'][0]):
            blk['c2p'] = ops.conv3x3_pack(blk['c2'][0])
        blocks.append(blk)
    if seam and dtype == ops.LP_DTYPE:
        for blk, nxt in zip(blocks[:-1], blocks[1:]):
            if ops.bottleneck_seam_supported(blk['c3'][0], nxt['c1'][0]):
                blk['seam'] = ops.bottleneck_seam_pack(blk['c3'][0], nxt['c1'][0])
                blk['seam_dims'] = (blk['c3'][0].shape[3], blk['c3'][0].shape[0], nxt['c1'][0].shape[0])
    return blocks


def pack_planes(blk):
    def true_w(pair):
        return ops.split16_true_weights(pair[0])

    w1, w2, w3 = true_w(blk['c1']), true_w(blk['c2']), true_w(blk['c3'])
    K1, K3c, mid, cout = w1.shape[3], w3.shape[3], w1.shape[0], w3.shape[0]
    if blk['stride'] != 1 or mid % 256 or cout % 256 or K1 % 128 or K3c % 128 or tuple(w2.shape[1:3]) != (3, 3) or w2.shape[3] % 64:
        return False
    p3 = {}
    t, u = ops.split16_plane_weights(w1.view(mid, K1), pair_first=True)
    p3['c1'] = (ops.conv1x1_pack(t), u, blk['c1'][1], mid)
    t, u = ops.split16_plane_weights(w2)
    p3['c2'] = (ops.conv3x3_pack(t), u, blk['c2'][1], w2.shape[0])
    if blk['ds'] is not None:
        if blk['ds_stride'] != 1:
            return False
        wd = true_w(blk['ds'])
        Kd = wd.shape[3]
        if Kd % 128:
            return False
        w, b = dual_weights(blk, wd, w3)
        t, u = ops.split16_plane_weights(w, segments=[Kd, K3c], pair_first=True)
        p3['dual'] = (ops.conv1x1_pack(t), u, b, cout)
    else:
        t, u = ops.split16_plane_weights(w3.view(cout, K3c))
        p3['c3'] = (ops.conv1x1_pack(t), u, blk['c3'][1], cout)
    blk['p3'] = p3
    return True


def fingerprint(model):
    return tuple((t.data_ptr(), t._version) for t in list(model.parameters()) + list(model.buffers()))


def pack_weights(model, device, precision, entries, where):
    ops.check_precision(precision)
    key = (device.index if device.index is not None else torch.cuda.current_device(), precision)
    cached = model._hip_packs.get(key)
    if cached is not None and (model.hip_static_weights or cached['fingerprint'] == fingerprint(model)):
        return cached
    first = next(model.parameters())
    if first.device != device:
        raise RuntimeError('model parameters live on {} but the input is on {}'.format(first.device, device))
    dtype = PRECISIONS[precision]
    s16 = precision == 'fp16x3'
    two = hasattr(model, 'layer4_1')
    with torch.no_grad():
        stem_w, stem_b = fold_conv_bn(model.conv1, model.bn1, torch.float32)
        pack = {
            'dtype': dtype,
            'stem': (stem_w, stem_b),
            'stem_lp': ops.pack_stem_weights_lp16(stem_w) if dtype == ops.LP_DTYPE else None,
            'stem_s16': ops.pack_stem_weights_split16(stem_w) if s16 else None,
            'trunk': pack_stage(model.layer1, dtype, split16=s16) + pack_stage(model.layer2, dtype, split16=s16) + pack_stage(model.layer3, dtype, seam=True, split16=s16),
        }
        for name in (('l4_1', 'l4_2') if two else ('l4',)):
            pack[name] = pack_stage(getattr(model, 'layer4' + name[2:]), dtype, split16=s16)
        stages = pack['trunk'] + (pack['l4_1'] + pack['l4_2'] if two else pack['l4'])
        entries(model, pack, dtype, s16)
        if s16:
            for blk in stages:
                for name in ('c1', 'c2', 'c3', 'ds'):
                    if blk.get(name) is not None and not (hasattr(blk[name][0], 'agrl_unscale') and getattr(blk[name][0], 'agrl_presplit', False)):
                        raise RuntimeError("fp16x3 pack: %s lost its pre-scale attributes" % name)
            if two and ops.split16_planes_available():
                first = len(model.layer1) + len(model.layer2) + 1
                pack['planes_from'] = first if all(pack_planes(blk) for blk in stages[first:]) else None
            for t in pack_tensors(pack):
                if hasattr(t, 'agrl_scaled'):
                    del t.agrl_scaled
    if dtype == ops.LP_DTYPE:
        check_packed_range(pack, where)
    pack['fingerprint'] = fingerprint(model)
    model._hip_packs[key] = pack
    return pack


def run_block_planes(x3, blk, pool=None):
    p3 = blk['p3']
    xp, rop = 1, 2
    y = ops.conv1x1_split16(x3, p3['c1'][0], p3['c1'][1], p3['c1'][2], p3['c1'][3], layout=xp)
    y = ops.conv3x3_split16(y, p3['c2'][0], p3['c2'][1], p3['c2'][2], p3['c2'][3])
    if 'dual' in p3:
        assert pool is None
        d = p3['dual']
        return ops.conv1x1_split16(x3, d[0], d[1], d[2], d[3], x2=y, layout=xp | rop)
    c = p3['c3']
    if pool is not None:
        return ops.conv1x1_split16_pool(y, c[0], c[1], c[2], c[3], x3, pool[0], pool[1], layout=rop)
    return ops.conv1x1_split16(y, c[0], c[1], c[2], c[3], residual3=x3, layout=rop)


def _conv2(y, blk):
    if 'c2p' in blk and y.shape[1] % 16 == 0 and y.shape[2] % 8 == 0:
        return ops.conv3x3_packed(y, blk['c2p'], blk['c2'][1], blk['c2'][0].shape[0], True)
    return ops.conv_bn_act(y, blk['c2'][0], blk['c2'][1], blk['stride'], 1, True)


def _conv1(x, blk):
    if 'c1p' in blk and x.is_contiguous():
        return ops.conv1x1_packed_res(x, blk['c1p'], blk['c1'][1], blk['c1'][0].shape[0], None, True)
    return ops.conv_bn_act(x, blk['c1'][0], blk['c1'][1], 1, 0, True)


def shortcut(x, blk):
    return x if blk['ds'] is None else ops.conv_bn_act(x, blk['ds'][0], blk['ds'][1], blk['ds_stride'], 0, False)


def run_block_inloop(x, blk, out_planes=0):
    y = ops.conv_bn_act(x, blk['c1'][0], blk['c1'][1], 1, 0, True, out_presplit=True)
    y = ops.conv_bn_act(y, blk['c2'][0], blk['c2'][1], blk['stride'], 1, True, x_presplit=True, out_presplit=True)
    if 'dual16' in blk and x.is_contiguous():
        return ops.conv1x1_dual_split16(x, y, blk['dual16'][0], blk['dual16'][1], blk['stride'], True, x2_presplit=True, out_planes=out_planes)
    out = ops.conv_bn_act(y, blk['c3'][0], blk['c3'][1], 1, 0, True, residual=shortcut(x, blk), x_presplit=True)
    return ops.to_split16_planes(out, out_planes) if out_planes else out


def is_inloop(blk):
    return getattr(blk['c1'][0], 'agrl_presplit', False)


def run_trunk(a, blocks):
    z = None
    for i, blk in enumerate(blocks):
        if is_inloop(blk):
            a = run_block_inloop(a, blk)
            continue
        nxt = blocks[i + 1] if i + 1 < len(blocks) else None
        y = z if z is not None else ops.conv_bn_act(a, blk['c1'][0], blk['c1'][1], 1, 0, True)
        if nxt is not None:
            ds = None if blk['ds'] is None else (blk['ds'][0], blk['ds_stride'])
            if ops.bottleneck_block_supported(y, blk['c2'][0], blk['stride'], blk['c3'][0], nxt['c1'][0], ds) and (
                    ds is None or a.shape[3] == 64):
                if ds is None:
                    a, z = ops.bottleneck_block(y, blk['c2'][0], blk['c2'][1], blk['c3'][0], blk['c3'][1], a,
                                                nxt['c1'][0], nxt['c1'][1])
                else:
                    a, z = ops.bottleneck_block(y, blk['c2'][0], blk['c2'][1], blk['c3'][0], blk['c3'][1], None,
                                                nxt['c1'][0], nxt['c1'][1], shortcut=(a, blk['ds'][0], blk['ds'][1]))
                continue
        y = _conv2(y, blk)
        fusable = nxt is not None and ops.bottleneck_tail_supported(y, blk['c3'][0], nxt['c1'][0])
        if fusable and blk['ds'] is not None and ops.bottleneck_tail_supported(
                y, blk['c3'][0], nxt['c1'][0], (blk['ds'][0], blk['ds_stride'])) and a.shape[3] == 64:
            a, z = ops.bottleneck_tail(y, blk['c3'][0], blk['c3'][1], None, nxt['c1'][0], nxt['c1'][1],
                                       shortcut=(a, blk['ds'][0], blk['ds'][1]))
            continue
        if ('dualps' in blk and a.is_contiguous() and y.is_contiguous() and a.dtype == y.dtype and a.shape[0] == y.shape[0]
                and tuple(y.shape[1:3]) == tuple((d - 1) // blk['stride'] + 1 for d in a.shape[1:3])):
            a = ops.conv1x1_packed_dual_strided(a, y, blk['dualps'], blk['dualps_bias'], blk['c3'][0].shape[0], blk['stride'], True)
            z = None
            continue
        sc = shortcut(a, blk)
        if nxt is not None and 'seam' in blk and (y.numel() // y.shape[-1]) % 128 == 0:
            a, z = ops.bottleneck_seam(y, blk['seam'], blk['c3'][1], sc, nxt['c1'][1], blk['seam_dims'])
            continue
        if fusable:
            a, z = ops.bottleneck_tail(y, blk['c3'][0], blk['c3'][1], sc, nxt['c1'][0], nxt['c1'][1])
        else:
            a = ops.conv_bn_act(y, blk['c3'][0], blk['c3'][1], 1, 0, True, residual=sc)
            z = None
    return a


def run_block(x, blk, pool=None):
    if is_inloop(blk):
        assert pool is None
        return run_block_inloop(x, blk)
    y = _conv1(x, blk)
    y = _conv2(y, blk)
    if (pool is None and 'dualp' in blk
            and x.shape[:3] == y.shape[:3] and x.dtype == y.dtype and x.is_contiguous() and y.is_contiguous()):
        return ops.conv1x1_packed(x, blk['dualp'], blk['dual'][1], blk['dual'][0].shape[0], True, x2=y, duo=True)
    if pool is None and 'dual' in blk and ops.conv1x1_dual_supported(x, y, blk['dual'][0]):
        return ops.conv1x1_dual(x, y, blk['dual'][0], blk['dual'][1], True)
    sc = shortcut(x, blk)
    duo = 'c3p' in blk and blk['ds'] is None and sc.is_contiguous() and y.is_contiguous()
    if pool is not None:
        if duo and tuple(y.shape[1:3]) == (16, 8):
            return ops.conv1x1_packed_res_pool(y, blk['c3p'], blk['c3'][1], blk['c3'][0].shape[0], sc, pool[0], pool[1], False)[0]
        return ops.conv1x1_bn_act_pool(y, blk['c3'][0], blk['c3'][1], sc, pool[0], pool[1], False)[0]
    if duo:
        return ops.conv1x1_packed_res(y, blk['c3p'], blk['c3'][1], blk['c3'][0].shape[0], sc)
    return ops.conv_bn_act(y, blk['c3'][0], blk['c3'][1], 1, 0, True, residual=sc)


def run_layer4(a, blocks, pool=None, planes=False):
    run = run_block_planes if planes else run_block
    for blk in blocks[:-1]:
        a = run(a, blk)
    return run(a, blocks[-1]) if pool is None else run(a, blocks[-1], pool=pool)


def run_stem(frames, pack, norm=None):
    mean, std = norm if norm is not None else (ops.PIXEL_MEAN, ops.PIXEL_STD)
    if pack['stem_lp'] is not None:
        return ops.stem_lp16(frames, pack['stem_lp'], pack['stem'][1], mean, std)
    if pack.get('stem_s16') is not None:
        return ops.stem_split16(frames, pack['stem_s16'][0], pack['stem_s16'][1], pack['stem_s16'][2], pack['stem'][1], mean, std)
    return ops.stem(frames, pack['stem'][0], pack['stem'][1], pack['dtype'], mean, std)


def eval_frames(model, x):
    if x.dtype == torch.uint8:
        _, B, S, _, _ = ops.clip_frames(x)
        norm = (getattr(model, 'pixel_mean', ops.PIXEL_MEAN), getattr(model, 'pixel_std', ops.PIXEL_STD))
        return x.reshape((B * S,) + tuple(x.shape[2:])), B, S, norm
    if x.dtype != torch.float32:
        raise TypeError('frames must be float32, got {}'.format(x.dtype))
    B, S, Cc, H, W = x.shape
    return x.reshape(B * S, Cc, H, W), B, S, None


def frame_size(frames):
    if frames.dtype == torch.uint8 and ops.frames_layout(frames.shape) == 'nhwc':
        return frames.shape[1], frames.shape[2]
    return frames.shape[2], frames.shape[3]


def single_bnneck(bn):
    a_bn = fold_bn1d(bn)
    return (torch.ones_like(a_bn[0]), torch.zeros_like(a_bn[1])), a_bn


def single_branch_tail(nodes, bnneck, B, S, P, hw):
    g_bn, a_bn = bnneck
    C = nodes.shape[-1]
    sqn = ops.row_sqnorm(nodes.view(B * S * P, C))
    gsum = torch.zeros((B * S, C), dtype=torch.float32, device=nodes.device)
    out = ops.attn_pool_bnneck(nodes, sqn, gsum, g_bn[0], g_bn[1], a_bn[0], a_bn[1], B, S, P, hw)
    return out[:, C:].contiguous()
```

### include/agrl_hip.h

```cpp
#ifndef AGRL_HIP_H
#define AGRL_HIP_H

#include <stddef.h>
#include <stdint.h>

#ifdef __cplusplus
extern "C" {
#endif

#define AGRL_F32 0
#define AGRL_LP16 1
#define AGRL_BF16 AGRL_LP16
#define AGRL_F32X3 2
#define AGRL_F32H3 3
#define AGRL_F32H3P 4

#define AGRL_METRIC_EUCLIDEAN 0
#define AGRL_METRIC_COSINE 1

typedef void* agrl_stream_t;

int agrl_version(void);
const char* agrl_last_error(void);

int agrl_lp16_is_f16(void);

int agrl_reload_options(void);
int agrl_built_with_ablation(void);


int agrl_stem_conv_bn_relu_maxpool(const float* x, const float* w, const float* bias, void* out,
                                   int N, int H, int W, int out_dtype, agrl_stream_t stream);

int agrl_stem_conv_bn_relu_maxpool_lp16(const float* x, const void* w_packed, const float* bias,
                                        void* out, int N, int H, int W, agrl_stream_t stream);

int agrl_stem_split16(const float* x, const void* wh_packed, const void* wl_packed, const float* bias, float* out, int N, int H,
                      int W, float w_unscale, agrl_stream_t stream);

#define AGRL_FRAMES_NCHW 0
#define AGRL_FRAMES_NHWC 1
int agrl_stem_conv_bn_relu_maxpool_u8(const unsigned char* x, const float* table, int layout, const float* w, const float* bias,
                                      void* out, int N, int H, int W, int out_dtype, agrl_stream_t stream);
int agrl_stem_conv_bn_relu_maxpool_lp16_u8(const unsigned char* x, const float* table, int layout, const void* w_packed,
                                           const float* bias, void* out, int N, int H, int W, agrl_stream_t stream);
int agrl_stem_split16_u8(const unsigned char* x, const float* table, int layout, const void* wh_packed, const void* wl_packed,
                         const float* bias, float* out, int N, int H, int W, float w_unscale, agrl_stream_t stream);

int agrl_frames_normalize_u8(const unsigned char* x, const float* table, int layout, float* out, int N, int H, int W,
                             agrl_stream_t stream);

int agrl_clip_resample_u8(const unsigned char* x, const int* geometry, unsigned char* out, int N, int Hs, int Ws, int OH, int OW,
                          agrl_stream_t stream);

int agrl_resample_taps_u8(int in, int out, int* k_out, int* bounds_out, agrl_stream_t stream);

int agrl_conv2d_bn_act(const void* x, const void* w, const float* bias, const void* residual,
                       void* out, int N, int H, int W, int Cin, int Cout, int R, int S, int stride,
                       int pad, int relu, int dtype, agrl_stream_t stream);

int agrl_conv2d_bn_act_split16(const void* x, const void* w_scaled, const float* bias, const void* residual, void* out, int N,
                               int H, int W, int Cin, int Cout, int R, int S, int stride, int pad, int relu, float w_unscale,
                               int x_presplit, int out_presplit, agrl_stream_t stream);

int agrl_split16_weights_inloop(const float* w_scaled, void* out, long long rows, int K, agrl_stream_t stream);

int agrl_conv1x1_dual_split16(const void* x, const void* x2, const void* w_scaled, const float* bias, void* out, int N, int H, int W,
                              int stride, int K1, int K2, int Cout, int relu, float w_unscale, int x2_presplit, int out_planes,
                              agrl_stream_t stream);

int agrl_split16_planes(const float* x, void* out, long long rows, int C, int nplanes, agrl_stream_t stream);
int agrl_split16_weight_planes(const float* x, void* out, long long rows, int C, float scale, agrl_stream_t stream);
int agrl_conv1x1_split16(const void* x, const void* packed, const float* bias, const void* residual, void* out, int M, int K3,
                         int Cout, int relu, float w_unscale, int layout, agrl_stream_t stream);
int agrl_conv1x1_split16_dual(const void* x, const void* x2, const void* packed, const float* bias, void* out, int M, int K1_3,
                              int K2_3, int Cout, int relu, float w_unscale, int layout, agrl_stream_t stream);
int agrl_conv1x1_split16_pool(const void* x, const void* packed, const float* bias, const void* residual, float* pool_out, int N,
                              int H, int W, int K3, int Cout, int relu, const int* splits, int n_splits, int mean, float w_unscale,
                              int layout, agrl_stream_t stream);
int agrl_conv3x3_packed_split16(const void* x, const void* packed, const float* bias, void* out, int N, int H, int W, int Cin3,
                                int Cout, int relu, float w_unscale, agrl_stream_t stream);

int agrl_conv1x1_dual_bn_act(const void* x1, const void* x2, const void* w, const float* bias, void* out, int M,
                             int K1, int K2, int Cout, int relu, agrl_stream_t stream);

int agrl_conv1x1_bn_act_pool(const void* x, const void* w, const float* bias, const void* residual,
                             void* out, float* pool_out, void* pool_out_lp, int N, int H, int W,
                             int Cin, int Cout, int relu, const int* splits, int n_splits, int mean,
                             agrl_stream_t stream);

int agrl_bottleneck_tail(const void* y2, const void* w3, const float* b3, const void* residual,
                         const void* x_short, const void* w_short, const float* b_short, void* out,
                         const void* w1_next, const float* b1_next, void* z, int M, int Cmid, int Cout,
                         int Cnext, int Cshort, agrl_stream_t stream);

long long agrl_bottleneck_seam_packed_bytes(int Cmid, int Cout, int Cnext);
int agrl_bottleneck_seam_pack(const void* w3, const void* w1_next, void* packed, int Cmid, int Cout, int Cnext,
                              agrl_stream_t stream);
int agrl_bottleneck_seam(const void* y2, const void* packed, const float* b3, const void* residual, void* out,
                         const float* b1_next, void* z, int M, int Cmid, int Cout, int Cnext, agrl_stream_t stream);

long long agrl_conv3x3_packed_bytes(int Cin, int Cout);
int agrl_conv3x3_pack(const void* w_ohwi, void* packed, int Cin, int Cout, agrl_stream_t stream);
int agrl_conv3x3_packed_bn_act(const void* x, const void* packed, const float* bias, void* out, int N, int H, int W, int Cin,
                               int Cout, int relu, agrl_stream_t stream);

long long agrl_conv1x1_packed_bytes(int K, int Cout);
int agrl_conv1x1_pack(const void* w, void* packed, int K, int Cout, agrl_stream_t stream);
int agrl_conv1x1_packed_bn_act(const void* x, const void* x2, const void* packed, const float* bias, void* out, int M, int K1,
                               int K2, int Cout, int relu, agrl_stream_t stream);

int agrl_conv1x1_packed_res_bn_act(const void* x, const void* packed, const float* bias, const void* residual, void* out, int M,
                                   int K, int Cout, int relu, agrl_stream_t stream);
int agrl_conv1x1_packed_res_pool(const void* x, const void* packed, const float* bias, const void* residual, float* pool_out,
                                 void* pool_out_lp, int N, int H, int W, int K, int Cout, int relu, const int* splits,
                                 int n_splits, int mean, agrl_stream_t stream);
int agrl_conv1x1_packed_dual_duo(const void* x, const void* x2, const void* packed, const float* bias, void* out, int M, int K1,
                                 int K2, int Cout, int relu, agrl_stream_t stream);
int agrl_conv1x1_packed_dual_strided(const void* x, const void* x2, const void* packed, const float* bias, void* out, int N, int Hi,
                                     int Wi, int stride, int K1, int K2, int Cout, int relu, agrl_stream_t stream);

int agrl_bottleneck_block(const void* z, const void* w2, const float* b2, const void* w3, const float* b3,
                          const void* residual, const void* x_short, const void* w_short, const float* b_short,
                          void* out, const void* w1_next, const float* b1_next, void* z_next, int F, int H, int W,
                          int Cmid, int Cout, int Cnext, agrl_stream_t stream);

int agrl_linear_nobias(const void* x, const void* w, float* y, int M, int K, int Nout,
                       int in_dtype, agrl_stream_t stream);


int agrl_pose_adjacency(const float* poses, const unsigned char* detected, float* adj, int B, int S,
                        int num_split, int pyramid_part, float height, float threshold, agrl_stream_t stream);
int agrl_pose_adjacency_bits(const float* poses, const unsigned char* detected, uint32_t* adj_bits, int B, int S, int num_split,
                             int pyramid_part, float height, float threshold, agrl_stream_t stream);
int agrl_adjacency_pack(const float* adj, uint32_t* adj_bits, int B, int V, agrl_stream_t stream);


int agrl_part_pool(const void* x4_1, const void* x4_2, float* gsum, float* nodes, void* nodes_lp,
                   int F, int h, int w, int C, const int* splits, int n_splits, int dtype,
                   agrl_stream_t stream);


int agrl_graph_gram(const float* f, float* gram_part, int B, int V, int C, int cslice,
                    agrl_stream_t stream);

int agrl_graph_finalize(const float* gram_part, int nz, const float* adj, float* G, int B, int V,
                        int use_pose, int learn_graph, int mask_diag, agrl_stream_t stream);
int agrl_graph_finalize_bits(const float* gram_part, int nz, const uint32_t* adj_bits, float* G, int B, int V, int use_pose,
                             int learn_graph, int mask_diag, agrl_stream_t stream);

int agrl_graph_apply(const float* G, const float* f, void* out, int out_dtype, int B, int V, int C, agrl_stream_t stream);
int agrl_graph_tracklet_operand(const float* f, const void* adj, int adj_packed, float* G_out, void* out, int out_dtype, int B,
                                int V, int C, int use_pose, int learn_graph, int mask_diag, agrl_stream_t stream);
int agrl_graph_linear_mix(const void* p_op, const void* w, const float* f, const float* bn_scale, const float* bn_shift,
                          float keep, float gamma, float slope, float* out, int M, int K, int Nout, int in_dtype,
                          agrl_stream_t stream);

int agrl_graph_propagate(const float* f, const float* h, const float* G, const float* bn_scale,
                         const float* bn_shift, float keep, float gamma, float slope, float* out, void* out_lp,
                         int B, int V, int C, agrl_stream_t stream);


int agrl_pam_pool(const void* x, const void* qk, float* xbar, float* xmean, int F, int h, int w, int C, int Cq,
                  const int* splits, int n_splits, int dtype, agrl_stream_t stream);

int agrl_pam_combine(const float* y, const float* bv, const float* xmean, float gamma, float* nodes, void* nodes_lp,
                     int rows, int C, agrl_stream_t stream);


int agrl_pam_pool_train(const float* x, const float* qk, float* xbar, float* xmean, float* abar, int F, int h, int w, int C,
                        int Cq, const int* splits, int n_splits, int dtype, agrl_stream_t stream);

int agrl_pam_pool_backward(const float* x, const float* qk, const float* dxbar, const float* dxmean, float* dx, float* dqk,
                           float* abar, int F, int h, int w, int C, int Cq, const int* splits, int n_splits, int dtype,
                           agrl_stream_t stream);

int agrl_pam_combine_train(const float* y, const float* bv, const float* xmean, const float* gamma, float* nodes, int rows, int C,
                           agrl_stream_t stream);

int agrl_pam_combine_backward(const float* dnodes, const float* y, const float* bv, const float* gamma, float* dy, float* dxmean,
                              float* dgamma, float* dbv, int rows, int C, void* workspace, size_t workspace_bytes,
                              agrl_stream_t stream);

size_t agrl_col_sum_workspace(int M, int C);
int agrl_col_sum(const float* x, float* out, int M, int C, void* workspace, size_t workspace_bytes, agrl_stream_t stream);


int agrl_row_sqnorm(const void* x, float* sqn, int R, int C, int dtype, agrl_stream_t stream);

int agrl_attn_pool_bnneck(const float* nodes, const float* sqn, const float* gsum,
                          const float* g_scale, const float* g_shift, const float* a_scale,
                          const float* a_shift, float* out, float* g_f, float* att_f, int B, int S,
                          int P, int C, int hw, agrl_stream_t stream);

int agrl_attn_tail(const float* nodes, const float* gsum, const float* g_scale, const float* g_shift, const float* a_scale,
                   const float* a_shift, float* out, float* g_f, float* att_f, float* node_sqn, float* out_sqn, void* q_lp,
                   float* q_f32, int B, int S, int P, int C, int hw, agrl_stream_t stream);

int agrl_clip_pool(const float* feats, float* out, int T, int n, int D, int mode, agrl_stream_t stream);

int agrl_clip_pool_ragged(const float* feats, const int* offsets, float* out, int* nonfinite, int N, int T, int D, int mode,
                          agrl_stream_t stream);


int agrl_sta_frame_stats(const void* map, float* vmean, float* nsum, float* nsq, int F, int h, int w, int C, int dtype,
                         agrl_stream_t stream);

#define AGRL_STA_MAP 0
#define AGRL_STA_NORM 1
int agrl_sta_fuse(const float* vmean, const float* nsum, const float* nsq, float* f_g, float* t_a, int32_t* idx, int B, int S, int C,
                  int h, int w, int mode, agrl_stream_t stream);

#define AGRL_LINEAR_BN_RELU_MAX_M 32
int agrl_linear_bn_relu(const float* x, const void* w, const float* scale, const float* shift, float* out, int M, int K, int N,
                        int w_dtype, agrl_stream_t stream);


int agrl_row_l2_normalize(const float* x, void* y, int R, int C, int ldy, int normalize, int out_dtype,
                          agrl_stream_t stream);

int agrl_distmat(const void* q, const void* g, const float* qn, const float* gn, float* dist,
                 int m, int n, int D, int ldd, int metric, int dtype, void* workspace,
                 size_t workspace_bytes, agrl_stream_t stream);

int agrl_distmat_split16(const void* q3, const void* g3, const float* qn, const float* gn, float* dist, int m, int n, int D3,
                         int ldd, int metric, float g_unscale, void* workspace, size_t workspace_bytes, agrl_stream_t stream);

int agrl_rank_topk(const float* dist, int m, int n, int ldd, int k, int idx_offset, int32_t* idx,
                   float* val, agrl_stream_t stream);

size_t agrl_distmat_topk_workspace(int m, int n);
int agrl_distmat_topk(const void* q, const void* g, const float* qn, const float* gn, int m, int n, int D, int metric,
                      int dtype, int k, int idx_offset, int32_t* idx, float* val, void* workspace,
                      size_t workspace_bytes, void* gemm_workspace, size_t gemm_workspace_bytes, agrl_stream_t stream);

int agrl_rank_argsort(const float* dist, int m, int n, int ldd, int32_t* idx, agrl_stream_t stream);

int agrl_rank_mars(const int32_t* topk_idx, const int32_t* q_pids, const int32_t* q_camids,
                   const int32_t* g_pids, const int32_t* g_camids, int m, int n, int k, double* ap,
                   float* cmc, agrl_stream_t stream);

int agrl_rank_market1501(const float* dist, int m, int n, int ldd, const int32_t* q_pids,
                         const int32_t* q_camids, const int32_t* g_pids, const int32_t* g_camids,
                         int max_rank, double* ap, float* cmc, int32_t* valid, agrl_stream_t stream);

size_t agrl_re_ranking_workspace(int m, int n, int k1);
int agrl_re_ranking(const float* q_g, const float* q_q, const float* g_g, int m, int n, int k1, int k2,
                    double lambda_value, float* final_dist, int ldf, void* workspace, size_t workspace_bytes,
                    agrl_stream_t stream);


size_t agrl_bn_workspace(int M, int C);

int agrl_bn_stats(const float* y, float* mean, float* var, int M, int C, void* workspace, size_t workspace_bytes,
                  agrl_stream_t stream);

int agrl_conv2d_stats(const float* x, const float* w, float* out, float* partial, size_t partial_bytes, int N, int H, int W, int Cin,
                      int Cout, int R, int S, int stride, int pad, int dtype, agrl_stream_t stream);
int agrl_bn_stats_from_partials(const float* partial, int rows, int C, int M, float* mean, float* var, void* workspace,
                                size_t workspace_bytes , agrl_stream_t stream);

int agrl_bn_fold_train(const float* mean, const float* var, const float* gamma, const float* beta, float eps, float momentum,
                       long long n, float* running_mean, float* running_var, long long* num_batches_tracked, float* scale,
                       float* shift, float* invstd, int C, agrl_stream_t stream);

int agrl_bn_apply(const float* y, const float* scale, const float* shift, const float* residual, float* out, unsigned char* mask,
                  int M, int C, int relu, float slope, agrl_stream_t stream);

int agrl_bn_backward(const float* dout, const float* out, const unsigned char* mask, const float* y, const float* mean,
                     const float* invstd, const float* gamma, int relu, float slope, float* dy, float* dz, float* dgamma,
                     float* dbeta, int M, int C, void* workspace, size_t workspace_bytes, agrl_stream_t stream);

int agrl_im2col_t(const float* x, float* T, int ldT, int F, int H, int W, int C, int R, int S, int stride, int pad,
                  agrl_stream_t stream);

int agrl_im2col_rows(const float* x, float* P, int ldP, int F, int H, int W, int C, int R, int S, int stride, int pad, int nchw,
                     agrl_stream_t stream);

int agrl_gemm_nt_splitk(const void* x, const void* w, float* y, int M, int K, int Nout, int in_dtype, void* workspace,
                        size_t workspace_bytes, agrl_stream_t stream);

size_t agrl_conv_wgrad_workspace(int F, int H, int W, int Cin, int Cout, int R, int S, int stride, int pad);
int agrl_conv_wgrad_plan(int F, int H, int W, int Cin, int Cout, int R, int S, int stride, int pad, int dtype, int* plan);
int agrl_conv_wgrad(const float* x, const float* dy, float* dw, int F, int H, int W, int Cin, int Cout, int R, int S, int stride,
                    int pad, int dtype, void* workspace, size_t workspace_bytes, agrl_stream_t stream);

int agrl_maxpool3x3s2(const float* x, float* out, unsigned char* idx, int F, int H, int W, int C, agrl_stream_t stream);
int agrl_maxpool3x3s2_backward(const float* dout, const unsigned char* idx, float* dx, int F, int H, int W, int C,
                               agrl_stream_t stream);


int agrl_axpby(const float* x, const float* y, float a, float b, float* out, size_t total, agrl_stream_t stream);

int agrl_part_pool_backward(const float* dg, const float* dnodes, float* dx1, float* dx2, int F, int S, int h, int w, int C,
                            const int* splits, int n_splits, agrl_stream_t stream);

int agrl_attn_pool_backward(const float* nodes, const float* datt, float* dnodes, int B, int S, int P, int C,
                            agrl_stream_t stream);

int agrl_graph_matrix_backward(const float* gram_part, int nz, const float* dG, float* M, int B, int V, int use_pose,
                               int mask_diag, agrl_stream_t stream);

int agrl_graph_pair_product(const float* a, const float* b, float* part, float* out, int B, int V, int C, agrl_stream_t stream);

int agrl_xent_label_smooth(const float* logits, const int32_t* targets, int n, int K, float eps, float* loss, float* dlogits,
                           float* row_loss, agrl_stream_t stream);


int agrl_triplet_hard_mine(const float* x, const int32_t* pids, int n, int d, float* dist_ap,
                           float* dist_an, int32_t* idx_ap, int32_t* idx_an, agrl_stream_t stream);


int agrl_diag_read_stream(const void* src, size_t bytes, float* sink, int workgroups, agrl_stream_t stream);

int agrl_triplet_loss(const float* x, const int32_t* pids, int n, int d, float margin, int soft, float* loss, float* grad,
                      float* dist_ap, float* dist_an, int32_t* idx_ap, int32_t* idx_an, float* coeff, agrl_stream_t stream);

int agrl_optim_geometry(int* chunk_elems, int* max_workgroups, int* descriptor_words);

int agrl_adam_step(const void* tensors, int n_tensors, const void* chunks, int n_chunks, float weight_decay,
                   float one_minus_beta1, float beta2, float one_minus_beta2, float step_size, float inv_sqrt_bc2, float eps,
                   int amsgrad, int zero_grad, agrl_stream_t stream);

int agrl_sgd_step(const void* tensors, int n_tensors, const void* chunks, int n_chunks, float weight_decay, float momentum,
                  float lr, int has_momentum, int first_step, int nesterov, int zero_grad, agrl_stream_t stream);

int agrl_rmsprop_step(const void* tensors, int n_tensors, const void* chunks, int n_chunks, float weight_decay, float alpha,
                      float one_minus_alpha, float eps, float momentum, float lr, int has_momentum, int zero_grad,
                      agrl_stream_t stream);

int agrl_adabound_step(const void* tensors, int n_tensors, const void* chunks, int n_chunks, float weight_decay,
                       float one_minus_beta1, float beta2, float one_minus_beta2, float step_size, float eps, float lower,
                       float upper, int amsbound, int zero_grad, agrl_stream_t stream);

int agrl_radam_step(const void* tensors, int n_tensors, const void* chunks, int n_chunks, float one_minus_beta1, float beta2,
                    float one_minus_beta2, float decay, float step_size, float eps, int adaptive, int zero_grad,
                    agrl_stream_t stream);

#ifdef __cplusplus
}
#endif
#endif
```

Measured before the change: 75550 frames/s.

## Chain consecutive layer3 bottleneck blocks into one persistent per-frame kernel

Adds a kernel that runs up to four stride-1 layer3 bottleneck blocks back to back inside one workgroup per frame. The 3x3 conv input patch stays in LDS and is refreshed by the seam epilogue, so the intermediate z maps never go to global memory and the separate conv3x3 and seam launches are dropped. The seam kernel body moves into a shared header so both kernels can use it. In exchange, parallelism is limited to one workgroup per frame, and the path is gated on frames >= CUs/2.

```diff
diff --git a/agrl.pytorch_amd/csrc/agrl_common.h b/agrl.pytorch_amd/csrc/agrl_common.h
--- a/agrl.pytorch_amd/csrc/agrl_common.h
+++ b/agrl.pytorch_amd/csrc/agrl_common.h
@@ -185,6 +185,7 @@
     int distmat_tile_n;
     int split16_ns;
     int duo_persist;
+    int l3_chain;
     int igemm_dbg, conv3x3_dbg;
 };
 const AgrlOpts& agrl_opts();
diff --git a/agrl.pytorch_amd/csrc/bottleneck_chain.hip b/agrl.pytorch_amd/csrc/bottleneck_chain.hip
--- /dev/null
+++ b/agrl.pytorch_amd/csrc/bottleneck_chain.hip
@@ -0,0 +1,196 @@
+#include "fat_dev.h"
+#include "seam_dev.h"
+
+namespace {
+
+struct ChainBlock {
+    const unsigned char* w2;
+    const float* b2;
+    const unsigned char* seam;
+    const float* b3;
+    const float* b1n;
+    const void* unused[3];
+};
+constexpr int CHAIN_MAX = 4;
+struct ChainParams {
+    const unsigned char* z1;
+    const ChainBlock* tab;
+    unsigned char* a[CHAIN_MAX + 1];
+    unsigned char* zout;
+    int n;
+};
+
+constexpr int CRING = 8;
+constexpr int CFPS = 9 * 2 * 4;
+constexpr int CPATCH = 23 * 1024;
+constexpr int CSLABS = 4;
+constexpr int CACC = 16;
+constexpr auto CHAIN_SCHED = fat_ring_sched<CRING, CFPS>([](int) { return 0; });
+constexpr int CHAIN_LDS = seam_lds_bytes<256, 1024>();
+static_assert(CSLABS * CPATCH <= CHAIN_LDS && CFPS % CRING == 0, "the patch fits where y2 and X live; a slab is whole ring turns");
+
+__global__ __launch_bounds__(NWV * 64) void bottleneck_chain_kernel(const ChainParams p) {
+    using std::integral_constant;
+    __shared__ __attribute__((aligned(16))) unsigned char smem_[CHAIN_LDS];
+    lds_u8_t* const smem = (lds_u8_t*)smem_;
+    const unsigned lds0 = (unsigned)(size_t)smem;
+
+    const int wave = __builtin_amdgcn_readfirstlane(threadIdx.x >> 6);
+    auto fresh_lane = [] {
+        unsigned l;
+        asm volatile("v_mbcnt_lo_u32_b32 %0, -1, 0\n\tv_mbcnt_hi_u32_b32 %0, -1, %0" : "=v"(l));
+        return (int)l;
+    };
+
+    {
+        const int lane = fresh_lane();
+        const unsigned char* zf = p.z1 + (size_t)blockIdx.x * (SBM * 256 * 2);
+        const unsigned char* zsrc = reinterpret_cast<const unsigned char*>(&g_zero16);
+#pragma unroll
+        for (int i = 0; i < 23; ++i) {
+            const int pi = wave + 4 * i;
+            const int slab = pi / 23, piece = pi - slab * 23;
+            const int row = piece * 8 + (lane >> 3);
+            const int py = row / 10, px = row - py * 10;
+            const bool ok = row < 180 && (unsigned)(py - 1) < 16u && (unsigned)(px - 1) < 8u;
+            const unsigned off = (unsigned)(((py - 1) * 8 + (px - 1)) * 512 + slab * 128 + (((lane & 7) ^ patch_g(py, px)) << 4));
+            fat_dma(ok ? zf + off : zsrc, __builtin_amdgcn_readfirstlane(lds0 + slab * CPATCH + piece * 1024));
+        }
+    }
+
+    asm volatile("" ::: "a255");
+    for (int i = 0; i < p.n; ++i) {
+        const ChainBlock blk = p.tab[i];
+        const int lane = fresh_lane();
+        const unsigned lane16 = (unsigned)lane * 16u;
+        const int frow = lane & 15, fchunk = lane >> 4;
+        const int fp = frag_px(frow);
+        int tbase[9];
+#pragma unroll
+        for (int t = 0; t < 9; ++t) tbase[t] = patch_off<10>((fp >> 3) + t / 3, (fp & 7) + t % 3, fchunk);
+
+        sfor<32>([&](auto qc) { fat_zero<CACC + decltype(qc)::value>(); });
+        const unsigned char* wstream = blk.w2 + (size_t)wave * CSLABS * (CFPS * 1024);
+        u32x4_t wr[CRING];
+        auto issue_w = [&](auto slot_c, const unsigned char* slab_base, auto pos_c) {
+            constexpr int SLOT = decltype(slot_c)::value, POS = decltype(pos_c)::value;
+            fat_gload<(POS & 3) * 1024>(wr[SLOT], lane16, slab_base + (POS & ~3) * 1024);
+        };
+        sfor<CRING>([&](auto ic) { issue_w(ic, wstream, ic); });
+        asm volatile("s_waitcnt vmcnt(%0)" ::"n"(CRING) : "memory");
+        wg_barrier();
+
+        u32x4_t xf[8];
+#pragma nounroll
+        for (int slab = 0; slab < CSLABS; ++slab) {
+            const unsigned char* ws = wstream + (size_t)slab * (CFPS * 1024);
+            const unsigned char* wsn = wstream + (size_t)(slab + 1 < CSLABS ? slab + 1 : 0) * (CFPS * 1024);
+            const lds_u8_t* sp = smem + slab * CPATCH;
+            auto ldx = [&](auto ks_c, auto b_c) {
+                constexpr int KS = decltype(ks_c)::value, B = decltype(b_c)::value;
+                return *reinterpret_cast<const lds_u32x4_t*>(sp + (tbase[KS >> 1] ^ ((KS & 1) * 64)) + B * 2560);
+            };
+            sfor<8>([&](auto bc) { xf[decltype(bc)::value] = ldx(integral_constant<int, 0>{}, bc); });
+            sfor<CFPS>([&](auto pc) {
+                constexpr int P = decltype(pc)::value;
+                constexpr int KS = P >> 2, A = P & 3, SL = P % CRING;
+                fat_wait<CHAIN_SCHED.allowed[P]>(wr[SL]);
+                sfor<8>([&](auto bc) {
+                    constexpr int B = decltype(bc)::value;
+                    fat_mfma<CACC + A * 8 + B>(wr[SL], xf[B]);
+                    if constexpr (A == 3 && KS + 1 < 18) {
+                        __builtin_amdgcn_sched_barrier(0);
+                        xf[B] = ldx(integral_constant<int, KS + 1>{}, bc);
+                    }
+                });
+                __builtin_amdgcn_sched_barrier(0);
+                constexpr int Q = P + CRING;
+                if constexpr (Q >= CFPS) issue_w(integral_constant<int, SL>{}, wsn, integral_constant<int, Q - CFPS>{});
+                else issue_w(integral_constant<int, SL>{}, ws, integral_constant<int, Q>{});
+            });
+        }
+        fat_ring_drain(wr);
+
+        wg_barrier();
+        {
+            const lds_u8_t* yw = smem + wave * 16384 + fp * 128;
+            const int sw = (fp >> 1) & 7;
+            sfor<2>([&](auto jc) {
+                constexpr int j = decltype(jc)::value;
+                const float4 b0 = *reinterpret_cast<const float4*>(blk.b2 + wave * 64 + 8 * fchunk + 32 * j);
+                const float4 b1 = *reinterpret_cast<const float4*>(blk.b2 + wave * 64 + 8 * fchunk + 32 * j + 4);
+                sfor<8>([&](auto bc) {
+                    constexpr int B = decltype(bc)::value;
+                    float v[8];
+                    fat_bias8<CACC + (2 * j) * 8 + B, CACC + (2 * j + 1) * 8 + B>(v, 1.f, b0, b1);
+                    fat_relu8(v, 1);
+                    const uint4 pk = fat_pack8(v);
+                    *reinterpret_cast<lds_u32x4_t*>(const_cast<lds_u8_t*>(yw) + B * 2048 + (((4 * j + fchunk) ^ sw) << 4)) = u32x4_t{pk.x, pk.y, pk.z, pk.w};
+                });
+            });
+        }
+        wg_barrier();
+
+        SeamParams sp;
+        sp.y2 = nullptr;
+        sp.wpk = blk.seam;
+        sp.b3 = blk.b3;
+        sp.res = i == 0 ? p.a[0] : i == 1 ? p.a[1] : i == 2 ? p.a[2] : p.a[3];
+        sp.out = i == 0 ? p.a[1] : i == 1 ? p.a[2] : i == 2 ? p.a[3] : p.a[4];
+        sp.b1n = blk.b1n;
+        sp.z = i + 1 == p.n ? p.zout : nullptr;
+        sp.M = 0;
+        const lds_u8_t* zw = smem + wave * CPATCH;
+        seam_tile<256, 1024, 256, true>(sp, smem, [&](auto jc, auto bc, const uint4& pk, int lane_z) {
+            constexpr int j = decltype(jc)::value, b = decltype(bc)::value;
+            const int frow = lane_z & 15, fchunk = lane_z >> 4;
+            *reinterpret_cast<lds_u32x4_t*>(const_cast<lds_u8_t*>(zw) + b * 2560 + patch_off<10>(1 + (frow >> 3), 1 + (frow & 7), 4 * j + fchunk)) =
+                u32x4_t{pk.x, pk.y, pk.z, pk.w};
+        });
+        for (int h = wave * 64 + fresh_lane(); h < CSLABS * 52 * 8; h += NWV * 64) {
+            const int hp = (h >> 3) % 52, slab = (h >> 3) / 52;
+            int py, px;
+            if (hp < 20) { py = hp < 10 ? 0 : 17; px = hp < 10 ? hp : hp - 10; }
+            else { py = 1 + ((hp - 20) >> 1); px = ((hp - 20) & 1) * 9; }
+            *reinterpret_cast<lds_u32x4_t*>(smem + slab * CPATCH + (py * 10 + px) * 128 + (h & 7) * 16) = u32x4_t{0u, 0u, 0u, 0u};
+        }
+    }
+}
+
+}
+
+extern "C" int agrl_bottleneck_chain_enabled(int frames) {
+    const int want = agrl_opts().l3_chain;
+    if (agrl_opt_set(want)) return want != 0;
+    return frames >= agrl_cu_count() / 2;
+}
+
+extern "C" int agrl_bottleneck_chain(const void* z1, const void* a0, const void* table, void* const* a_out, void* z_out, int frames, int n,
+                                     agrl_stream_t stream) {
+    AGRL_CHECK_ARG(z1 && a0 && table && a_out && z_out, "agrl_bottleneck_chain: null pointer");
+    AGRL_CHECK_ARG(n >= 1 && n <= CHAIN_MAX, "agrl_bottleneck_chain: 1 to %d chained blocks, got %d", CHAIN_MAX, n);
+    AGRL_CHECK_ARG(frames > 0 && (size_t)frames * SBM * 1024 * 2 < (1ull << 32), "agrl_bottleneck_chain: maps beyond 4 GB are not addressed");
+    ChainParams p;
+    p.z1 = reinterpret_cast<const unsigned char*>(z1);
+    p.tab = reinterpret_cast<const ChainBlock*>(table);
+    for (int i = 0; i <= CHAIN_MAX; ++i) p.a[i] = nullptr;
+    p.a[0] = reinterpret_cast<unsigned char*>(const_cast<void*>(a0));
+    for (int i = 0; i < n; ++i) p.a[i + 1] = reinterpret_cast<unsigned char*>(a_out[i]);
+    p.zout = reinterpret_cast<unsigned char*>(z_out);
+    p.n = n;
+    const size_t abytes = (size_t)frames * SBM * 1024 * 2;
+    uintptr_t al = (uintptr_t)z1 | (uintptr_t)table | (uintptr_t)z_out;
+    for (int i = 0; i <= n; ++i) {
+        AGRL_CHECK_ARG(p.a[i], "agrl_bottleneck_chain: null pointer");
+        al |= (uintptr_t)p.a[i];
+        for (int k = 0; k < i; ++k) {
+            const uintptr_t lo = (uintptr_t)p.a[i] < (uintptr_t)p.a[k] ? (uintptr_t)p.a[i] : (uintptr_t)p.a[k];
+            const uintptr_t hi = (uintptr_t)p.a[i] < (uintptr_t)p.a[k] ? (uintptr_t)p.a[k] : (uintptr_t)p.a[i];
+            AGRL_CHECK_ARG(hi - lo >= abytes, "agrl_bottleneck_chain: the residual-stream buffers must not overlap");
+        }
+    }
+    AGRL_CHECK_ARG((al & 15) == 0, "agrl_bottleneck_chain: pointers must be 16-byte aligned");
+    hipLaunchKernelGGL(bottleneck_chain_kernel, dim3(frames), dim3(NWV * 64), 0, (hipStream_t)stream, p);
+    AGRL_CHECK_LAUNCH("agrl_bottleneck_chain");
+    return 0;
+}
diff --git a/agrl.pytorch_amd/csrc/bottleneck_seam.hip b/agrl.pytorch_amd/csrc/bottleneck_seam.hip
--- a/agrl.pytorch_amd/csrc/bottleneck_seam.hip
+++ b/agrl.pytorch_amd/csrc/bottleneck_seam.hip
@@ -1,374 +1,11 @@
-#include <utility>
-
-#include "igemm_dev.h"
+#include "seam_dev.h"
 
 namespace {
 
-struct SeamParams {
-    const unsigned char* y2;
-    const unsigned char* wpk;
-    const float* b3;
-    const unsigned char* res;
-    unsigned char* out;
-    const float* b1n;
-    unsigned char* z;
-    int M;
-};
-
-#ifndef SEAM_ABL
-#define SEAM_ABL 0
-#endif
-constexpr int SBM = 128;
-constexpr int SCH = 256;
-
-template <typename F, int... Is>
-__device__ __forceinline__ void static_for_impl(F&& f, std::integer_sequence<int, Is...>) {
-    (f(std::integral_constant<int, Is>{}), ...);
-}
-template <int N, typename F>
-__device__ __forceinline__ void static_for(F&& f) {
-    static_for_impl(f, std::make_integer_sequence<int, N>{});
-}
-
-typedef unsigned u32x4_t __attribute__((ext_vector_type(4)));
-typedef __attribute__((address_space(3))) unsigned char lds_u8_t;
-typedef __attribute__((address_space(3))) u32x4_t lds_u32x4_t;
-__device__ __forceinline__ u32x4_t lds_ld16(const lds_u8_t* p) {
-#if SEAM_ABL & 16
-    return u32x4_t{(unsigned)(size_t)p, 1u, 2u, 3u};
-#else
-    return *reinterpret_cast<const lds_u32x4_t*>(p);
-#endif
-}
-
-template <int IMM>
-__device__ __forceinline__ void gload16_asm(u32x4_t& dst, unsigned off, const unsigned char* base) {
-    static_assert(IMM >= 0 && IMM < 4096, "13-bit signed immediate");
-    asm volatile("global_load_dwordx4 %0, %1, %2 offset:%3" : "=v"(dst) : "v"(off), "s"(base), "n"(IMM) : "memory");
-}
-template <int RQ>
-__device__ __forceinline__ void mfma_v(f32x4_t& acc, const u32x4_t& b) {
-    if constexpr (kLpF16) asm volatile("v_mfma_f32_16x16x32_f16 %0, a[%c2:%c3], %1, %0" : "+v"(acc) : "v"(b), "n"(4 * RQ), "n"(4 * RQ + 3));
-    else asm volatile("v_mfma_f32_16x16x32_bf16 %0, a[%c2:%c3], %1, %0" : "+v"(acc) : "v"(b), "n"(4 * RQ), "n"(4 * RQ + 3));
-}
-template <int AQ, int RQ>
-__device__ __forceinline__ void mfma_a(const u32x4_t& b) {
-    if constexpr (kLpF16)
-        asm volatile("v_mfma_f32_16x16x32_f16 a[%c1:%c2], a[%c3:%c4], %0, a[%c1:%c2]" ::"v"(b), "n"(4 * AQ), "n"(4 * AQ + 3), "n"(4 * RQ), "n"(4 * RQ + 3));
-    else
-        asm volatile("v_mfma_f32_16x16x32_bf16 a[%c1:%c2], a[%c3:%c4], %0, a[%c1:%c2]" ::"v"(b), "n"(4 * AQ), "n"(4 * AQ + 3), "n"(4 * RQ), "n"(4 * RQ + 3));
-}
-template <int AQ>
-__device__ __forceinline__ void acc_zero() {
-    asm volatile("v_accvgpr_write_b32 a[%c0], 0\n\tv_accvgpr_write_b32 a[%c1], 0\n\tv_accvgpr_write_b32 a[%c2], 0\n\tv_accvgpr_write_b32 a[%c3], 0" ::"n"(4 * AQ),
-                 "n"(4 * AQ + 1), "n"(4 * AQ + 2), "n"(4 * AQ + 3));
-}
-template <int AQ>
-__device__ __forceinline__ f32x4_t acc_read() {
-    float x, y, z, w;
-    asm volatile("v_accvgpr_read_b32 %0, a[%c4]\n\tv_accvgpr_read_b32 %1, a[%c5]\n\tv_accvgpr_read_b32 %2, a[%c6]\n\tv_accvgpr_read_b32 %3, a[%c7]"
-                 : "=v"(x), "=v"(y), "=v"(z), "=v"(w)
-                 : "n"(4 * AQ), "n"(4 * AQ + 1), "n"(4 * AQ + 2), "n"(4 * AQ + 3));
-    return f32x4_t{x, y, z, w};
-}
-template <int IMM>
-__device__ __forceinline__ void gstore16_asm(const u32x4_t& v, unsigned off, unsigned char* base) {
-    asm volatile("global_store_dwordx4 %0, %1, %2 offset:%3\n\ts_nop 1" ::"v"(off), "v"(v), "s"(base), "n"(IMM) : "memory");
-}
-template <int RQ, int IMM>
-__device__ __forceinline__ void ring_load(unsigned off, const unsigned char* base) {
-    static_assert(IMM >= 0 && IMM < 4096, "13-bit signed immediate");
-    asm volatile("global_load_dwordx4 a[%c2:%c3], %0, %1 offset:%4" ::"v"(off), "s"(base), "n"(4 * RQ), "n"(4 * RQ + 3), "n"(IMM) : "memory");
-}
-__device__ __forceinline__ void mfma_drain() { asm volatile("s_nop 15\n\ts_nop 15" ::: "memory"); }
-
-__device__ __forceinline__ void dma16s(const unsigned char* sbase, unsigned voff, unsigned lds_wave_addr) {
-    unsigned keep;
-    asm volatile(
-        "s_mov_b32 %0, m0\n\ts_mov_b32 m0, %3\n\ts_nop 0\n\tglobal_load_lds_dwordx4 %1, %2\n\ts_mov_b32 m0, %0"
-        : "=&s"(keep)
-        : "v"(voff), "s"(sbase), "s"(lds_wave_addr)
-        : "memory");
-}
-
-constexpr int NWV = 4;
-constexpr int FW1 = 4;
-constexpr int Y2P = 4;
-constexpr int S_OPS = (SEAM_ABL & 1) ? 0 : 32;
-template <int KS1, int FW2, bool Y2RING, int RING>
-struct Sched {
-    static constexpr int G1F = FW1 * KS1, G2F = 8 * FW2, FPC = G1F + G2F;
-    int allowed[FPC];
-};
-template <int KS1, int FW2, bool Y2RING, int RING>
-constexpr Sched<KS1, FW2, Y2RING, RING> make_sched() {
-    using S = Sched<KS1, FW2, Y2RING, RING>;
-    S s{};
-    int issued[4][S::FPC] = {};
-    int seq = 0;
-    for (int p = 0; p < RING; ++p) issued[0][p] = seq++;
-    for (int k = 0; k < 3; ++k) {
-        for (int p = 0; p < S::FPC; ++p) {
-            if (p == S::G1F) seq += S_OPS;
-            if (k == 1) s.allowed[p] = seq - 1 - issued[k][p];
-            if (Y2RING && p < S::G1F && (p % FW1) == FW1 - 1 && ((p / FW1) & 1)) seq += Y2P;
-            const int q = p + RING;
-            if (q >= S::FPC) issued[k + 1][q - S::FPC] = seq++;
-            else issued[k][q] = seq++;
-        }
-    }
-    return s;
-}
-template <int KS1, int FW2, bool Y2RING, int RING>
-struct SchedOf {
-    static constexpr Sched<KS1, FW2, Y2RING, RING> value = make_sched<KS1, FW2, Y2RING, RING>();
-};
-
 template <int K1, int N1, int N2>
 __global__ __launch_bounds__(NWV * 64) void bottleneck_seam_kernel(const SeamParams p) {
-    static_assert((K1 == 256 || K1 == 512) && N1 % SCH == 0 && (N2 == 256 || N2 == 512), "shapes");
-    constexpr int NC = N1 / SCH;
-    constexpr int KS1 = K1 / 32;
-    constexpr int FW2 = N2 / 64;
-    constexpr bool Y2RING = K1 > 256;
-    constexpr int NKT = K1 / 64;
-    constexpr int NSL = 5, AHEAD = 3;
-    constexpr int XO = Y2RING ? NSL * 16384 : 64 * 1024;
-    constexpr int BIAS_OFF = XO + 64 * 1024;
-    constexpr int RING = N2 == 256 ? 16 : 8;
-    constexpr int NA2 = (64 - RING) < FW2 * 8 ? (64 - RING) : FW2 * 8;
-    constexpr int NV2 = FW2 * 8 - NA2;
-    using SCHED = SchedOf<KS1, FW2, Y2RING, RING>;
-    constexpr int G1F = FW1 * KS1, G2F = 8 * FW2, FPC = G1F + G2F;
-    static_assert(FPC % RING == 0, "the ring index of a fragment must not depend on the chunk");
-
-    __shared__ __attribute__((aligned(16))) unsigned char smem_[BIAS_OFF + N1 * 4];
-    lds_u8_t* const smem = (lds_u8_t*)smem_;
-    const unsigned lds0 = (unsigned)(size_t)smem;
-
-    const int tid = threadIdx.x;
-    const int lane = tid & 63;
-    const int wave = __builtin_amdgcn_readfirstlane(tid >> 6);
-    const int frow = lane & 15, fchunk = lane >> 4;
-    const int m0 = blockIdx.x * SBM;
-    const unsigned lane16 = (unsigned)lane * 16u;
-
-    unsigned a_off[2];
-#pragma unroll
-    for (int j = 0; j < 2; ++j) {
-        const int row = wave * 32 + j * 8 + (lane >> 3);
-        a_off[j] = (unsigned)(m0 + row) * (K1 * 2) + (unsigned)(((lane & 7) ^ ((row >> 1) & 7)) << 4);
-    }
-    const unsigned ldsA = __builtin_amdgcn_readfirstlane(lds0 + wave * 4096);
-    auto issue_y2 = [&](int kt, int slot) {
-        const unsigned char* src = p.y2 + kt * 128;
-        const unsigned dst = ldsA + slot * 16384;
-        dma16s(src, a_off[0], dst);
-        dma16s(src, a_off[1], dst + 1024);
-        dma16s(src + 16 * (K1 * 2), a_off[0], dst + 2048);
-        dma16s(src + 16 * (K1 * 2), a_off[1], dst + 3072);
-    };
-    const int lo128 = frow * 128 + ((fchunk ^ ((frow >> 1) & 7)) << 4);
-    const unsigned r_off = (unsigned)(m0 + frow) * (N1 * 2) + (unsigned)(wave * 64 + 8 * fchunk) * 2;
-
-    const lds_u8_t* xptr = smem + XO + lane16;
-    const lds_u8_t* sa0 = smem + lo128;
-    const lds_u8_t* sa1 = smem + (lo128 ^ 64);
-    asm volatile("" : "+v"(xptr), "+v"(sa0), "+v"(sa1));
-
-    auto issue_w = [&](auto slot_c, const unsigned char* chunk_base, auto pos_c) {
-        constexpr int SLOT = decltype(slot_c)::value, POS = decltype(pos_c)::value;
-        if constexpr (SEAM_ABL & 8) return;
-        ring_load<SLOT, (POS & 3) * 1024>(lane16, chunk_base + (POS & ~3) * 1024);
-    };
-    auto chunk_stream = [&](int c) { return p.wpk + (size_t)(c * NWV + wave) * (FPC * 1024); };
-
-    f32x4_t acc1[FW1][8];
-    asm volatile("" ::: "a255");
-    static_for<NA2>([&](auto qc) { acc_zero<RING + decltype(qc)::value>(); });
-    f32x4_t acc2v[NV2 > 0 ? NV2 : 1];
-#pragma unroll
-    for (int i = 0; i < (NV2 > 0 ? NV2 : 1); ++i) acc2v[i] = f32x4_t{0.f, 0.f, 0.f, 0.f};
-
-    u32x4_t rres[8][2];
-    auto load_residual = [&](int c) {
-        const unsigned char* rc = p.res + (size_t)c * (SCH * 2);
-#pragma unroll
-        for (int b = 0; b < 8; ++b) {
-            if constexpr (SEAM_ABL & 1) { rres[b][0] = u32x4_t{(unsigned)c, r_off, 1u, 2u}; rres[b][1] = rres[b][0]; continue; }
-            gload16_asm<0>(rres[b][0], r_off, rc + b * (16 * N1 * 2));
-            gload16_asm<64>(rres[b][1], r_off, rc + b * (16 * N1 * 2));
-        }
-    };
-    auto init_acc1 = [&](int c) {
-#pragma unroll
-        for (int j = 0; j < 2; ++j) {
-            float bias[8];
-            {
-                const lds_u8_t* bs = smem + BIAS_OFF + (c * SCH + wave * 64 + 32 * j + 8 * fchunk) * 4;
-                const u32x4_t b0 = *reinterpret_cast<const lds_u32x4_t*>(bs), b1 = *reinterpret_cast<const lds_u32x4_t*>(bs + 16);
-#pragma unroll
-                for (int e = 0; e < 4; ++e) { bias[e] = __uint_as_float(b0[e]); bias[4 + e] = __uint_as_float(b1[e]); }
-            }
-#pragma unroll
-            for (int b = 0; b < 8; ++b) {
-                const uint32_t w4[4] = {rres[b][j][0], rres[b][j][1], rres[b][j][2], rres[b][j][3]};
-                float v[8];
-#pragma unroll
-                for (int e = 0; e < 4; ++e) unpack_lp16x2(w4[e], v[2 * e], v[2 * e + 1]);
-#pragma unroll
-                for (int e = 0; e < 8; ++e) v[e] = (SEAM_ABL & 1) ? bias[e] : v[e] + bias[e];
-                acc1[2 * j][b] = f32x4_t{v[0], v[1], v[2], v[3]};
-                acc1[2 * j + 1][b] = f32x4_t{v[4], v[5], v[6], v[7]};
-                __builtin_amdgcn_sched_barrier(0);
-            }
-        }
-    };
-
-    using std::integral_constant;
-
-    load_residual(0);
-#pragma unroll
-    for (int i = 0; i < N1 / 1024; ++i)
-        dma16s(reinterpret_cast<const unsigned char*>(p.b3) + (wave * (N1 / 1024) + i) * 1024, lane16, lds0 + BIAS_OFF + (wave * (N1 / 1024) + i) * 1024);
-#pragma unroll
-    for (int t = 0; t < (Y2RING ? AHEAD : NKT); ++t) issue_y2(t, t);
-    {
-        const unsigned char* s0 = chunk_stream(0);
-        static_for<RING>([&](auto ic) { issue_w(ic, s0, ic); });
-    }
-    asm volatile("s_waitcnt vmcnt(%0)" ::"n"((SEAM_ABL & 8) ? 0 : RING) : "memory");
-    __builtin_amdgcn_s_barrier();
-    asm volatile("" ::: "memory");
-
-    u32x4_t bf[8];
-    int kt_slot = 0;
-    int slot_off = 0;
-    auto ld_y2 = [&](auto ks_c, int b) {
-        constexpr int KS = decltype(ks_c)::value;
-        const lds_u8_t* base = (KS & 1) ? sa1 : sa0;
-        if constexpr (Y2RING) return lds_ld16(base + slot_off + b * 2048);
-        else return lds_ld16(base + (KS >> 1) * 16384 + b * 2048);
-    };
-
-    for (int c = 0;; ++c) {
-        const bool last = c + 1 == NC;
-        const int cn = last ? 0 : c + 1;
-        const unsigned char* ws = chunk_stream(c);
-        const unsigned char* wsn = chunk_stream(cn);
-
-#pragma unroll
-        for (int b = 0; b < 8; ++b) asm volatile("" : "+v"(rres[b][0]), "+v"(rres[b][1]));
-        init_acc1(c);
-        __builtin_amdgcn_sched_barrier(0);
-#pragma unroll
-        for (int b = 0; b < 8; ++b) bf[b] = ld_y2(integral_constant<int, 0>{}, b);
-        asm volatile("s_nop 4" ::: "memory");
-
-        static_for<FPC>([&](auto pc) {
-            constexpr int P = decltype(pc)::value;
-            constexpr bool G1 = P < G1F;
-            constexpr int F = G1 ? P : P - G1F;
-            constexpr int FW = G1 ? FW1 : FW2;
-            constexpr int KS = F / FW, A = F % FW;
-            constexpr int SL = P % RING;
-            constexpr bool LAST_A = A + 1 == FW;
-
-            if constexpr (P == G1F) {
-                if constexpr (!Y2RING) {
-                    __builtin_amdgcn_s_barrier();
-                    asm volatile("" ::: "memory");
-                }
-                mfma_drain();
-                unsigned char* oc = p.out + (size_t)c * (SCH * 2);
-                const lds_u8_t* xw = xptr + wave * 16384;
-                static_for<2>([&](auto jc) {
-                    constexpr int j = decltype(jc)::value;
-#pragma unroll
-                    for (int b = 0; b < 8; ++b) {
-                        float v[8];
-#pragma unroll
-                        for (int e = 0; e < 4; ++e) {
-                            v[e] = relu_nan(acc1[2 * j][b][e]);
-                            v[4 + e] = relu_nan(acc1[2 * j + 1][b][e]);
-                        }
-                        const u32x4_t pk = {pack_lp16x2(v[0], v[1]), pack_lp16x2(v[2], v[3]), pack_lp16x2(v[4], v[5]), pack_lp16x2(v[6], v[7])};
-                        if constexpr (!(SEAM_ABL & 1)) gstore16_asm<j * 64>(pk, r_off, oc + b * (16 * N1 * 2));
-                        *reinterpret_cast<lds_u32x4_t*>(const_cast<lds_u8_t*>(xw) + (j * 8 + b) * 1024) = pk;
-                    }
-                });
-                load_residual(cn);
-                wg_barrier();
-#pragma unroll
-                for (int b = 0; b < 8; ++b) bf[b] = lds_ld16(xptr + b * 1024);
-            }
-
-            if constexpr (!(SEAM_ABL & 8)) wait_vmcnt<SCHED::value.allowed[P]>();
-
-            if constexpr (Y2RING && G1 && LAST_A && (KS & 1)) {
-                __builtin_amdgcn_s_barrier();
-                asm volatile("" ::: "memory");
-                const int nslot = (kt_slot + (KS >> 1) + 1) % NSL;
-                issue_y2(((KS >> 1) + AHEAD) % NKT, (nslot + AHEAD - 1) % NSL);
-                slot_off = nslot * 16384;
-            }
-            static_for<8>([&](auto bc) {
-                constexpr int b = decltype(bc)::value;
-                if constexpr (G1) {
-                    if constexpr (SEAM_ABL & 2) asm volatile("" ::"v"(bf[b]));
-                    else mfma_v<SL>(acc1[A][b], bf[b]);
-                } else {
-                    if constexpr (SEAM_ABL & 4) asm volatile("" ::"v"(bf[b]));
-                    else if constexpr (A * 8 + b < NA2) mfma_a<RING + A * 8 + b, SL>(bf[b]);
-                    else mfma_v<SL>(acc2v[A * 8 + b - NA2], bf[b]);
-                }
-                if constexpr (LAST_A) {
-                    if constexpr (G1 && KS + 1 < KS1) {
-                        __builtin_amdgcn_sched_barrier(0);
-                        bf[b] = ld_y2(integral_constant<int, KS + 1>{}, b);
-                    } else if constexpr (!G1 && KS + 1 < 8) {
-                        __builtin_amdgcn_sched_barrier(0);
-                        bf[b] = lds_ld16(xptr + ((KS + 1) * 8 + b) * 1024);
-                    }
-                }
-            });
-            __builtin_amdgcn_sched_barrier(0);
-            constexpr int Q = P + RING;
-            if constexpr (Q >= FPC) issue_w(integral_constant<int, SL>{}, wsn, integral_constant<int, Q - FPC>{});
-            else issue_w(integral_constant<int, SL>{}, ws, integral_constant<int, Q>{});
-            if constexpr (Y2RING && P + 1 == G1F) kt_slot = (kt_slot + NKT) % NSL;
-        });
-        if (last) break;
-    }
-    asm volatile("s_waitcnt vmcnt(0)" ::: "memory");
-    mfma_drain();
-
-    unsigned lane_z;
-    asm volatile("v_mbcnt_lo_u32_b32 %0, -1, 0\n\tv_mbcnt_hi_u32_b32 %0, -1, %0" : "=v"(lane_z));
-    const int frow_z = lane_z & 15, fchunk_z = lane_z >> 4;
-    lp16_t* __restrict__ zp = reinterpret_cast<lp16_t*>(p.z);
-    const int cb2 = wave * (N2 / NWV) + 8 * fchunk_z;
-    static_for<FW2 / 2>([&](auto jc) {
-        constexpr int j = decltype(jc)::value;
-        const float4 b0 = *reinterpret_cast<const float4*>(p.b1n + cb2 + 32 * j);
-        const float4 b1 = *reinterpret_cast<const float4*>(p.b1n + cb2 + 32 * j + 4);
-        static_for<8>([&](auto bc) {
-            constexpr int b = decltype(bc)::value;
-            const int gm = m0 + b * 16 + frow_z;
-            f32x4_t lo, hi;
-            if constexpr ((2 * j) * 8 + b < NA2) lo = acc_read<RING + (2 * j) * 8 + b>();
-            else lo = acc2v[(2 * j) * 8 + b - NA2];
-            if constexpr ((2 * j + 1) * 8 + b < NA2) hi = acc_read<RING + (2 * j + 1) * 8 + b>();
-            else hi = acc2v[(2 * j + 1) * 8 + b - NA2];
-            float v[8];
-            v[0] = lo[0] + b0.x; v[1] = lo[1] + b0.y; v[2] = lo[2] + b0.z; v[3] = lo[3] + b0.w;
-            v[4] = hi[0] + b1.x; v[5] = hi[1] + b1.y; v[6] = hi[2] + b1.z; v[7] = hi[3] + b1.w;
-#pragma unroll
-            for (int e = 0; e < 8; ++e) v[e] = relu_nan(v[e]);
-            *reinterpret_cast<uint4*>(zp + (size_t)gm * N2 + cb2 + 32 * j) =
-                make_uint4(pack_lp16x2(v[0], v[1]), pack_lp16x2(v[2], v[3]), pack_lp16x2(v[4], v[5]), pack_lp16x2(v[6], v[7]));
-        });
-    });
+    __shared__ __attribute__((aligned(16))) unsigned char smem_[seam_lds_bytes<K1, N1>()];
+    seam_tile<K1, N1, N2, false>(p, (lds_u8_t*)smem_, 0);
 }
 
 __global__ void seam_pack_kernel(const lp16_t* __restrict__ w3, const lp16_t* __restrict__ w1n, uint4* __restrict__ wpk, int K1, int N1, int N2) {
diff --git a/agrl.pytorch_amd/csrc/common.hip b/agrl.pytorch_amd/csrc/common.hip
--- a/agrl.pytorch_amd/csrc/common.hip
+++ b/agrl.pytorch_amd/csrc/common.hip
@@ -58,6 +58,7 @@
     o.conv3x3_fat_pb = opt_int("AGRL_CONV3X3_FAT_PB");
     o.conv3x3_half = opt_int("AGRL_CONV3X3_HALF");
     o.conv3x3_half_stagger = opt_int("AGRL_CONV3X3_HALF_STAGGER");
+    o.l3_chain = opt_int("AGRL_L3_CHAIN");
 #ifdef AGRL_ABLATE
     o.igemm_dbg = agrl_opt_set(opt_int("AGRL_IGEMM_DBG")) ? opt_int("AGRL_IGEMM_DBG") : 0;
     o.conv3x3_dbg = agrl_opt_set(opt_int("AGRL_CONV3X3_DBG")) ? opt_int("AGRL_CONV3X3_DBG") : 0;
diff --git a/agrl.pytorch_amd/csrc/seam_dev.h b/agrl.pytorch_amd/csrc/seam_dev.h
--- /dev/null
+++ b/agrl.pytorch_amd/csrc/seam_dev.h
@@ -0,0 +1,387 @@
+#pragma once
+#include <utility>
+
+#include "igemm_dev.h"
+
+namespace {
+
+struct SeamParams {
+    const unsigned char* y2;
+    const unsigned char* wpk;
+    const float* b3;
+    const unsigned char* res;
+    unsigned char* out;
+    const float* b1n;
+    unsigned char* z;
+    int M;
+};
+
+#ifndef SEAM_ABL
+#define SEAM_ABL 0
+#endif
+constexpr int SBM = 128;
+constexpr int SCH = 256;
+
+template <typename F, int... Is>
+__device__ __forceinline__ void static_for_impl(F&& f, std::integer_sequence<int, Is...>) {
+    (f(std::integral_constant<int, Is>{}), ...);
+}
+template <int N, typename F>
+__device__ __forceinline__ void static_for(F&& f) {
+    static_for_impl(f, std::make_integer_sequence<int, N>{});
+}
+
+typedef unsigned u32x4_t __attribute__((ext_vector_type(4)));
+typedef __attribute__((address_space(3))) unsigned char lds_u8_t;
+typedef __attribute__((address_space(3))) u32x4_t lds_u32x4_t;
+__device__ __forceinline__ u32x4_t lds_ld16(const lds_u8_t* p) {
+#if SEAM_ABL & 16
+    return u32x4_t{(unsigned)(size_t)p, 1u, 2u, 3u};
+#else
+    return *reinterpret_cast<const lds_u32x4_t*>(p);
+#endif
+}
+
+template <int IMM>
+__device__ __forceinline__ void gload16_asm(u32x4_t& dst, unsigned off, const unsigned char* base) {
+    static_assert(IMM >= 0 && IMM < 4096, "13-bit signed immediate");
+    asm volatile("global_load_dwordx4 %0, %1, %2 offset:%3" : "=v"(dst) : "v"(off), "s"(base), "n"(IMM) : "memory");
+}
+template <int RQ>
+__device__ __forceinline__ void mfma_v(f32x4_t& acc, const u32x4_t& b) {
+    if constexpr (kLpF16) asm volatile("v_mfma_f32_16x16x32_f16 %0, a[%c2:%c3], %1, %0" : "+v"(acc) : "v"(b), "n"(4 * RQ), "n"(4 * RQ + 3));
+    else asm volatile("v_mfma_f32_16x16x32_bf16 %0, a[%c2:%c3], %1, %0" : "+v"(acc) : "v"(b), "n"(4 * RQ), "n"(4 * RQ + 3));
+}
+template <int AQ, int RQ>
+__device__ __forceinline__ void mfma_a(const u32x4_t& b) {
+    if constexpr (kLpF16)
+        asm volatile("v_mfma_f32_16x16x32_f16 a[%c1:%c2], a[%c3:%c4], %0, a[%c1:%c2]" ::"v"(b), "n"(4 * AQ), "n"(4 * AQ + 3), "n"(4 * RQ), "n"(4 * RQ + 3));
+    else
+        asm volatile("v_mfma_f32_16x16x32_bf16 a[%c1:%c2], a[%c3:%c4], %0, a[%c1:%c2]" ::"v"(b), "n"(4 * AQ), "n"(4 * AQ + 3), "n"(4 * RQ), "n"(4 * RQ + 3));
+}
+template <int AQ>
+__device__ __forceinline__ void acc_zero() {
+    asm volatile("v_accvgpr_write_b32 a[%c0], 0\n\tv_accvgpr_write_b32 a[%c1], 0\n\tv_accvgpr_write_b32 a[%c2], 0\n\tv_accvgpr_write_b32 a[%c3], 0" ::"n"(4 * AQ),
+                 "n"(4 * AQ + 1), "n"(4 * AQ + 2), "n"(4 * AQ + 3));
+}
+template <int AQ>
+__device__ __forceinline__ f32x4_t acc_read() {
+    float x, y, z, w;
+    asm volatile("v_accvgpr_read_b32 %0, a[%c4]\n\tv_accvgpr_read_b32 %1, a[%c5]\n\tv_accvgpr_read_b32 %2, a[%c6]\n\tv_accvgpr_read_b32 %3, a[%c7]"
+                 : "=v"(x), "=v"(y), "=v"(z), "=v"(w)
+                 : "n"(4 * AQ), "n"(4 * AQ + 1), "n"(4 * AQ + 2), "n"(4 * AQ + 3));
+    return f32x4_t{x, y, z, w};
+}
+template <int IMM>
+__device__ __forceinline__ void gstore16_asm(const u32x4_t& v, unsigned off, unsigned char* base) {
+    asm volatile("global_store_dwordx4 %0, %1, %2 offset:%3\n\ts_nop 1" ::"v"(off), "v"(v), "s"(base), "n"(IMM) : "memory");
+}
+template <int RQ, int IMM>
+__device__ __forceinline__ void ring_load(unsigned off, const unsigned char* base) {
+    static_assert(IMM >= 0 && IMM < 4096, "13-bit signed immediate");
+    asm volatile("global_load_dwordx4 a[%c2:%c3], %0, %1 offset:%4" ::"v"(off), "s"(base), "n"(4 * RQ), "n"(4 * RQ + 3), "n"(IMM) : "memory");
+}
+__device__ __forceinline__ void mfma_drain() { asm volatile("s_nop 15\n\ts_nop 15" ::: "memory"); }
+
+__device__ __forceinline__ void dma16s(const unsigned char* sbase, unsigned voff, unsigned lds_wave_addr) {
+    unsigned keep;
+    asm volatile(
+        "s_mov_b32 %0, m0\n\ts_mov_b32 m0, %3\n\ts_nop 0\n\tglobal_load_lds_dwordx4 %1, %2\n\ts_mov_b32 m0, %0"
+        : "=&s"(keep)
+        : "v"(voff), "s"(sbase), "s"(lds_wave_addr)
+        : "memory");
+}
+
+constexpr int NWV = 4;
+constexpr int FW1 = 4;
+constexpr int Y2P = 4;
+constexpr int S_OPS = (SEAM_ABL & 1) ? 0 : 32;
+template <int KS1, int FW2, bool Y2RING, int RING>
+struct Sched {
+    static constexpr int G1F = FW1 * KS1, G2F = 8 * FW2, FPC = G1F + G2F;
+    int allowed[FPC];
+};
+template <int KS1, int FW2, bool Y2RING, int RING>
+constexpr Sched<KS1, FW2, Y2RING, RING> make_sched() {
+    using S = Sched<KS1, FW2, Y2RING, RING>;
+    S s{};
+    int issued[4][S::FPC] = {};
+    int seq = 0;
+    for (int p = 0; p < RING; ++p) issued[0][p] = seq++;
+    for (int k = 0; k < 3; ++k) {
+        for (int p = 0; p < S::FPC; ++p) {
+            if (p == S::G1F) seq += S_OPS;
+            if (k == 1) s.allowed[p] = seq - 1 - issued[k][p];
+            if (Y2RING && p < S::G1F && (p % FW1) == FW1 - 1 && ((p / FW1) & 1)) seq += Y2P;
+            const int q = p + RING;
+            if (q >= S::FPC) issued[k + 1][q - S::FPC] = seq++;
+            else issued[k][q] = seq++;
+        }
+    }
+    return s;
+}
+template <int KS1, int FW2, bool Y2RING, int RING>
+struct SchedOf {
+    static constexpr Sched<KS1, FW2, Y2RING, RING> value = make_sched<KS1, FW2, Y2RING, RING>();
+};
+
+template <int K1, int N1>
+constexpr int seam_lds_bytes() { return (K1 > 256 ? 5 * 16384 : 64 * 1024) + 64 * 1024 + N1 * 4; }
+
+template <int K1, int N1, int N2, bool CHAIN, typename ZPIECE>
+__device__ __forceinline__ void seam_tile(const SeamParams& p, lds_u8_t* const smem, ZPIECE&& zpiece) {
+    static_assert((K1 == 256 || K1 == 512) && N1 % SCH == 0 && (N2 == 256 || N2 == 512), "shapes");
+    static_assert(!CHAIN || K1 == 256, "the chained form needs the resident y2 tile");
+    constexpr int NC = N1 / SCH;
+    constexpr int KS1 = K1 / 32;
+    constexpr int FW2 = N2 / 64;
+    constexpr bool Y2RING = K1 > 256;
+    constexpr int NKT = K1 / 64;
+    constexpr int NSL = 5, AHEAD = 3;
+    constexpr int XO = Y2RING ? NSL * 16384 : 64 * 1024;
+    constexpr int BIAS_OFF = XO + 64 * 1024;
+    constexpr int RING = N2 == 256 ? 16 : 8;
+    constexpr int NA2 = (64 - RING) < FW2 * 8 ? (64 - RING) : FW2 * 8;
+    constexpr int NV2 = FW2 * 8 - NA2;
+    using SCHED = SchedOf<KS1, FW2, Y2RING, RING>;
+    constexpr int G1F = FW1 * KS1, G2F = 8 * FW2, FPC = G1F + G2F;
+    static_assert(FPC % RING == 0, "the ring index of a fragment must not depend on the chunk");
+    static_assert(BIAS_OFF + N1 * 4 == seam_lds_bytes<K1, N1>(), "the caller's LDS array");
+
+    const unsigned lds0 = (unsigned)(size_t)smem;
+
+    const int tid = threadIdx.x;
+    const int lane = tid & 63;
+    const int wave = __builtin_amdgcn_readfirstlane(tid >> 6);
+    const int frow = lane & 15, fchunk = lane >> 4;
+    const int m0 = blockIdx.x * SBM;
+    const unsigned lane16 = (unsigned)lane * 16u;
+
+    unsigned a_off[2];
+#pragma unroll
+    for (int j = 0; j < 2; ++j) {
+        const int row = wave * 32 + j * 8 + (lane >> 3);
+        a_off[j] = (unsigned)(m0 + row) * (K1 * 2) + (unsigned)(((lane & 7) ^ ((row >> 1) & 7)) << 4);
+    }
+    const unsigned ldsA = __builtin_amdgcn_readfirstlane(lds0 + wave * 4096);
+    auto issue_y2 = [&](int kt, int slot) {
+        const unsigned char* src = p.y2 + kt * 128;
+        const unsigned dst = ldsA + slot * 16384;
+        dma16s(src, a_off[0], dst);
+        dma16s(src, a_off[1], dst + 1024);
+        dma16s(src + 16 * (K1 * 2), a_off[0], dst + 2048);
+        dma16s(src + 16 * (K1 * 2), a_off[1], dst + 3072);
+    };
+    const int lo128 = frow * 128 + ((fchunk ^ ((frow >> 1) & 7)) << 4);
+    const unsigned r_off = (unsigned)(m0 + frow) * (N1 * 2) + (unsigned)(wave * 64 + 8 * fchunk) * 2;
+
+    const lds_u8_t* xptr = smem + XO + lane16;
+    const lds_u8_t* sa0 = smem + lo128;
+    const lds_u8_t* sa1 = smem + (lo128 ^ 64);
+    asm volatile("" : "+v"(xptr), "+v"(sa0), "+v"(sa1));
+
+    auto issue_w = [&](auto slot_c, const unsigned char* chunk_base, auto pos_c) {
+        constexpr int SLOT = decltype(slot_c)::value, POS = decltype(pos_c)::value;
+        if constexpr (SEAM_ABL & 8) return;
+        ring_load<SLOT, (POS & 3) * 1024>(lane16, chunk_base + (POS & ~3) * 1024);
+    };
+    auto chunk_stream = [&](int c) { return p.wpk + (size_t)(c * NWV + wave) * (FPC * 1024); };
+
+    f32x4_t acc1[FW1][8];
+    asm volatile("" ::: "a255");
+    static_for<NA2>([&](auto qc) { acc_zero<RING + decltype(qc)::value>(); });
+    f32x4_t acc2v[NV2 > 0 ? NV2 : 1];
+#pragma unroll
+    for (int i = 0; i < (NV2 > 0 ? NV2 : 1); ++i) acc2v[i] = f32x4_t{0.f, 0.f, 0.f, 0.f};
+
+    u32x4_t rres[8][2];
+    auto load_residual = [&](int c) {
+        const unsigned char* rc = p.res + (size_t)c * (SCH * 2);
+#pragma unroll
+        for (int b = 0; b < 8; ++b) {
+            if constexpr (SEAM_ABL & 1) { rres[b][0] = u32x4_t{(unsigned)c, r_off, 1u, 2u}; rres[b][1] = rres[b][0]; continue; }
+            gload16_asm<0>(rres[b][0], r_off, rc + b * (16 * N1 * 2));
+            gload16_asm<64>(rres[b][1], r_off, rc + b * (16 * N1 * 2));
+        }
+    };
+    auto init_acc1 = [&](int c) {
+#pragma unroll
+        for (int j = 0; j < 2; ++j) {
+            float bias[8];
+            {
+                const lds_u8_t* bs = smem + BIAS_OFF + (c * SCH + wave * 64 + 32 * j + 8 * fchunk) * 4;
+                const u32x4_t b0 = *reinterpret_cast<const lds_u32x4_t*>(bs), b1 = *reinterpret_cast<const lds_u32x4_t*>(bs + 16);
+#pragma unroll
+                for (int e = 0; e < 4; ++e) { bias[e] = __uint_as_float(b0[e]); bias[4 + e] = __uint_as_float(b1[e]); }
+            }
+#pragma unroll
+            for (int b = 0; b < 8; ++b) {
+                const uint32_t w4[4] = {rres[b][j][0], rres[b][j][1], rres[b][j][2], rres[b][j][3]};
+                float v[8];
+#pragma unroll
+                for (int e = 0; e < 4; ++e) unpack_lp16x2(w4[e], v[2 * e], v[2 * e + 1]);
+#pragma unroll
+                for (int e = 0; e < 8; ++e) v[e] = (SEAM_ABL & 1) ? bias[e] : v[e] + bias[e];
+                acc1[2 * j][b] = f32x4_t{v[0], v[1], v[2], v[3]};
+                acc1[2 * j + 1][b] = f32x4_t{v[4], v[5], v[6], v[7]};
+                __builtin_amdgcn_sched_barrier(0);
+            }
+        }
+    };
+
+    using std::integral_constant;
+
+    load_residual(0);
+#pragma unroll
+    for (int i = 0; i < N1 / 1024; ++i)
+        dma16s(reinterpret_cast<const unsigned char*>(p.b3) + (wave * (N1 / 1024) + i) * 1024, lane16, lds0 + BIAS_OFF + (wave * (N1 / 1024) + i) * 1024);
+    if constexpr (!CHAIN) {
+#pragma unroll
+        for (int t = 0; t < (Y2RING ? AHEAD : NKT); ++t) issue_y2(t, t);
+    }
+    {
+        const unsigned char* s0 = chunk_stream(0);
+        static_for<RING>([&](auto ic) { issue_w(ic, s0, ic); });
+    }
+    asm volatile("s_waitcnt vmcnt(%0)" ::"n"((SEAM_ABL & 8) ? 0 : RING) : "memory");
+    __builtin_amdgcn_s_barrier();
+    asm volatile("" ::: "memory");
+
+    u32x4_t bf[8];
+    int kt_slot = 0;
+    int slot_off = 0;
+    auto ld_y2 = [&](auto ks_c, int b) {
+        constexpr int KS = decltype(ks_c)::value;
+        const lds_u8_t* base = (KS & 1) ? sa1 : sa0;
+        if constexpr (Y2RING) return lds_ld16(base + slot_off + b * 2048);
+        else return lds_ld16(base + (KS >> 1) * 16384 + b * 2048);
+    };
+
+    for (int c = 0;; ++c) {
+        const bool last = c + 1 == NC;
+        const int cn = last ? 0 : c + 1;
+        const unsigned char* ws = chunk_stream(c);
+        const unsigned char* wsn = chunk_stream(cn);
+
+#pragma unroll
+        for (int b = 0; b < 8; ++b) asm volatile("" : "+v"(rres[b][0]), "+v"(rres[b][1]));
+        init_acc1(c);
+        __builtin_amdgcn_sched_barrier(0);
+#pragma unroll
+        for (int b = 0; b < 8; ++b) bf[b] = ld_y2(integral_constant<int, 0>{}, b);
+        asm volatile("s_nop 4" ::: "memory");
+
+        static_for<FPC>([&](auto pc) {
+            constexpr int P = decltype(pc)::value;
+            constexpr bool G1 = P < G1F;
+            constexpr int F = G1 ? P : P - G1F;
+            constexpr int FW = G1 ? FW1 : FW2;
+            constexpr int KS = F / FW, A = F % FW;
+            constexpr int SL = P % RING;
+            constexpr bool LAST_A = A + 1 == FW;
+
+            if constexpr (P == G1F) {
+                if constexpr (!Y2RING) {
+                    __builtin_amdgcn_s_barrier();
+                    asm volatile("" ::: "memory");
+                }
+                mfma_drain();
+                unsigned char* oc = p.out + (size_t)c * (SCH * 2);
+                const lds_u8_t* xw = xptr + wave * 16384;
+                static_for<2>([&](auto jc) {
+                    constexpr int j = decltype(jc)::value;
+#pragma unroll
+                    for (int b = 0; b < 8; ++b) {
+                        float v[8];
+#pragma unroll
+                        for (int e = 0; e < 4; ++e) {
+                            v[e] = relu_nan(acc1[2 * j][b][e]);
+                            v[4 + e] = relu_nan(acc1[2 * j + 1][b][e]);
+                        }
+                        const u32x4_t pk = {pack_lp16x2(v[0], v[1]), pack_lp16x2(v[2], v[3]), pack_lp16x2(v[4], v[5]), pack_lp16x2(v[6], v[7])};
+                        if constexpr (!(SEAM_ABL & 1)) gstore16_asm<j * 64>(pk, r_off, oc + b * (16 * N1 * 2));
+                        *reinterpret_cast<lds_u32x4_t*>(const_cast<lds_u8_t*>(xw) + (j * 8 + b) * 1024) = pk;
+                    }
+                });
+                load_residual(cn);
+                wg_barrier();
+#pragma unroll
+                for (int b = 0; b < 8; ++b) bf[b] = lds_ld16(xptr + b * 1024);
+            }
+
+            if constexpr (!(SEAM_ABL & 8)) wait_vmcnt<SCHED::value.allowed[P]>();
+
+            if constexpr (Y2RING && G1 && LAST_A && (KS & 1)) {
+                __builtin_amdgcn_s_barrier();
+                asm volatile("" ::: "memory");
+                const int nslot = (kt_slot + (KS >> 1) + 1) % NSL;
+                issue_y2(((KS >> 1) + AHEAD) % NKT, (nslot + AHEAD - 1) % NSL);
+                slot_off = nslot * 16384;
+            }
+            static_for<8>([&](auto bc) {
+                constexpr int b = decltype(bc)::value;
+                if constexpr (G1) {
+                    if constexpr (SEAM_ABL & 2) asm volatile("" ::"v"(bf[b]));
+                    else mfma_v<SL>(acc1[A][b], bf[b]);
+                } else {
+                    if constexpr (SEAM_ABL & 4) asm volatile("" ::"v"(bf[b]));
+                    else if constexpr (A * 8 + b < NA2) mfma_a<RING + A * 8 + b, SL>(bf[b]);
+                    else mfma_v<SL>(acc2v[A * 8 + b - NA2], bf[b]);
+                }
+                if constexpr (LAST_A) {
+                    if constexpr (G1 && KS + 1 < KS1) {
+                        __builtin_amdgcn_sched_barrier(0);
+                        bf[b] = ld_y2(integral_constant<int, KS + 1>{}, b);
+                    } else if constexpr (!G1 && KS + 1 < 8) {
+                        __builtin_amdgcn_sched_barrier(0);
+                        bf[b] = lds_ld16(xptr + ((KS + 1) * 8 + b) * 1024);
+                    }
+                }
+            });
+            __builtin_amdgcn_sched_barrier(0);
+            constexpr int Q = P + RING;
+            if constexpr (Q >= FPC) issue_w(integral_constant<int, SL>{}, wsn, integral_constant<int, Q - FPC>{});
+            else issue_w(integral_constant<int, SL>{}, ws, integral_constant<int, Q>{});
+            if constexpr (Y2RING && P + 1 == G1F) kt_slot = (kt_slot + NKT) % NSL;
+        });
+        if (last) break;
+    }
+    asm volatile("s_waitcnt vmcnt(0)" ::: "memory");
+    mfma_drain();
+    if constexpr (CHAIN) wg_barrier();
+
+    unsigned lane_z;
+    asm volatile("v_mbcnt_lo_u32_b32 %0, -1, 0\n\tv_mbcnt_hi_u32_b32 %0, -1, %0" : "=v"(lane_z));
+    const int frow_z = lane_z & 15, fchunk_z = lane_z >> 4;
+    lp16_t* __restrict__ zp = reinterpret_cast<lp16_t*>(p.z);
+    const int cb2 = wave * (N2 / NWV) + 8 * fchunk_z;
+    static_for<FW2 / 2>([&](auto jc) {
+        constexpr int j = decltype(jc)::value;
+        const float4 b0 = *reinterpret_cast<const float4*>(p.b1n + cb2 + 32 * j);
+        const float4 b1 = *reinterpret_cast<const float4*>(p.b1n + cb2 + 32 * j + 4);
+        static_for<8>([&](auto bc) {
+            constexpr int b = decltype(bc)::value;
+            const int gm = m0 + b * 16 + frow_z;
+            f32x4_t lo, hi;
+            if constexpr ((2 * j) * 8 + b < NA2) lo = acc_read<RING + (2 * j) * 8 + b>();
+            else lo = acc2v[(2 * j) * 8 + b - NA2];
+            if constexpr ((2 * j + 1) * 8 + b < NA2) hi = acc_read<RING + (2 * j + 1) * 8 + b>();
+            else hi = acc2v[(2 * j + 1) * 8 + b - NA2];
+            float v[8];
+            v[0] = lo[0] + b0.x; v[1] = lo[1] + b0.y; v[2] = lo[2] + b0.z; v[3] = lo[3] + b0.w;
+            v[4] = hi[0] + b1.x; v[5] = hi[1] + b1.y; v[6] = hi[2] + b1.z; v[7] = hi[3] + b1.w;
+#pragma unroll
+            for (int e = 0; e < 8; ++e) v[e] = relu_nan(v[e]);
+            if constexpr (CHAIN) {
+                const uint4 pk = make_uint4(pack_lp16x2(v[0], v[1]), pack_lp16x2(v[2], v[3]), pack_lp16x2(v[4], v[5]), pack_lp16x2(v[6], v[7]));
+                zpiece(jc, bc, pk, (int)lane_z);
+                if (p.z) *reinterpret_cast<uint4*>(zp + (size_t)gm * N2 + cb2 + 32 * j) = pk;
+            } else {
+                *reinterpret_cast<uint4*>(zp + (size_t)gm * N2 + cb2 + 32 * j) =
+                    make_uint4(pack_lp16x2(v[0], v[1]), pack_lp16x2(v[2], v[3]), pack_lp16x2(v[4], v[5]), pack_lp16x2(v[6], v[7]));
+            }
+        });
+    });
+}
+
+}
diff --git a/agrl.pytorch_amd/torchreid/_hip.py b/agrl.pytorch_amd/torchreid/_hip.py
--- a/agrl.pytorch_amd/torchreid/_hip.py
+++ b/agrl.pytorch_amd/torchreid/_hip.py
@@ -65,6 +65,8 @@
     "agrl_bottleneck_seam_packed_bytes": [_i, _i, _i],
     "agrl_bottleneck_seam_pack": [_p, _p, _p, _i, _i, _i, _p],
     "agrl_bottleneck_seam": [_p, _p, _p, _p, _p, _p, _p, _i, _i, _i, _i, _p],
+    "agrl_bottleneck_chain_enabled": [_i],
+    "agrl_bottleneck_chain": [_p, _p, _p, _p, _p, _i, _i, _p],
     "agrl_conv3x3_packed_bytes": [_i, _i],
     "agrl_conv1x1_packed_bytes": [_i, _i],
     "agrl_conv1x1_pack": [_p, _p, _i, _i, _p],
diff --git a/agrl.pytorch_amd/torchreid/hip_ops.py b/agrl.pytorch_amd/torchreid/hip_ops.py
--- a/agrl.pytorch_amd/torchreid/hip_ops.py
+++ b/agrl.pytorch_amd/torchreid/hip_ops.py
@@ -638,6 +638,51 @@
         call("agrl_bottleneck_seam", ptr(y2), ptr(packed), ptr(b3), ptr(residual), ptr(out), ptr(b1_next), ptr(z), M, Cmid, Cout,
              Cnext, _stream(y2))
     return out, z
+
+
+CHAIN_MAX = 4
+
+
+def bottleneck_chain_table(blocks):
+    rows = [[b['c2p'].data_ptr(), b['c2'][1].data_ptr(), b['seam'].data_ptr(), b['c3'][1].data_ptr(), b['seam_b1n'].data_ptr(), 0, 0, 0]
+            for b in blocks]
+    return torch.tensor(rows, dtype=torch.int64).to(blocks[0]['c2p'].device)
+
+
+def bottleneck_chain_block_ok(blk):
+    return ('c2p' in blk and 'seam' in blk and 'seam_b1n' in blk and blk['ds'] is None and blk['stride'] == 1
+            and blk.get('seam_dims') == (256, 1024, 256) and tuple(blk['c2'][0].shape) == (256, 3, 3, 256)
+            and blk['c2'][0].dtype == LP_DTYPE)
+
+
+def bottleneck_chain_supported(z, a, blocks, forced=False):
+    if not (1 <= len(blocks) <= CHAIN_MAX and all(bottleneck_chain_block_ok(b) for b in blocks)):
+        return False
+    if not (z.dtype == LP_DTYPE and a.dtype == LP_DTYPE and z.dim() == 4 and tuple(z.shape[1:]) == (16, 8, 256)
+            and tuple(a.shape) == (z.shape[0], 16, 8, 1024) and z.is_contiguous() and a.is_contiguous()):
+        return False
+    return forced or bool(_hip.lib().agrl_bottleneck_chain_enabled(int(z.shape[0])))
+
+
+def bottleneck_chain(z, a, table, n, work=None, out=None):
+    F = z.shape[0]
+    assert 1 <= n <= CHAIN_MAX and table.dtype == torch.int64 and tuple(table.shape[1:]) == (8,) and table.shape[0] >= n
+    assert z.dtype == LP_DTYPE and a.dtype == LP_DTYPE and tuple(z.shape) == (F, 16, 8, 256) and tuple(a.shape) == (F, 16, 8, 1024)
+    assert z.is_contiguous() and a.is_contiguous()
+    if work is None:
+        work = [torch.empty_like(a) for _ in range(n - 1)]
+    assert len(work) >= n - 1 and all(w.dtype == a.dtype and w.numel() == a.numel() and w.is_contiguous() for w in work[:n - 1])
+    out = torch.empty_like(a) if out is None else out
+    assert out.dtype == a.dtype and out.numel() == a.numel() and out.is_contiguous()
+    zn = torch.empty_like(z)
+    bufs = (C.c_void_p * n)(*([ptr(w) for w in work[:n - 1]] + [ptr(out)]))
+    if _hip.PROFILE is not None:
+        M = F * 128
+        _hip.PROFILE_TAG = {"flops": 2.0 * M * n * (9 * 256 * 256 + 2 * 256 * 1024),
+                            "bytes": 2.0 * (z.numel() + zn.numel() + (2 * n) * a.numel()) + n * 2.0 * (9 * 256 * 256 + 2 * 256 * 1024)}
+    with _dev(z):
+        call("agrl_bottleneck_chain", ptr(z), ptr(a), ptr(table), bufs, ptr(zn), F, n, _stream(z))
+    return out, zn
 
 
 def conv3x3_packed_enabled():
diff --git a/agrl.pytorch_amd/torchreid/models/_resnet_hip.py b/agrl.pytorch_amd/torchreid/models/_resnet_hip.py
--- a/agrl.pytorch_amd/torchreid/models/_resnet_hip.py
+++ b/agrl.pytorch_amd/torchreid/models/_resnet_hip.py
@@ -108,7 +108,21 @@
             if ops.bottleneck_seam_supported(blk['c3'][0], nxt['c1'][0]):
                 blk['seam'] = ops.bottleneck_seam_pack(blk['c3'][0], nxt['c1'][0])
                 blk['seam_dims'] = (blk['c3'][0].shape[3], blk['c3'][0].shape[0], nxt['c1'][0].shape[0])
+                blk['seam_b1n'] = nxt['c1'][1]
+        i = 0
+        while i < len(blocks):
+            run = chain_run(blocks, i)
+            if run:
+                blocks[i]['chain'] = (run, ops.bottleneck_chain_table(blocks[i:i + run]))
+            i += max(run, 1)
     return blocks
+
+
+def chain_run(blocks, i):
+    n = 0
+    while i + n < len(blocks) and n < ops.CHAIN_MAX and ops.bottleneck_chain_block_ok(blocks[i + n]):
+        n += 1
+    return n
 
 
 def pack_planes(blk):
@@ -234,12 +248,21 @@
 
 def run_trunk(a, blocks):
     z = None
+    skip = 0
     for i, blk in enumerate(blocks):
+        if skip:
+            skip -= 1
+            continue
         if is_inloop(blk):
             a = run_block_inloop(a, blk)
             continue
         nxt = blocks[i + 1] if i + 1 < len(blocks) else None
         y = z if z is not None else ops.conv_bn_act(a, blk['c1'][0], blk['c1'][1], 1, 0, True)
+        if 'chain' in blk and ops.bottleneck_chain_supported(y, a, blocks[i:i + blk['chain'][0]]):
+            n, table = blk['chain']
+            a, z = ops.bottleneck_chain(y, a, table, n)
+            skip = n - 1
+            continue
         if nxt is not None:
             ds = None if blk['ds'] is None else (blk['ds'][0], blk['ds_stride'])
             if ops.bottleneck_block_supported(y, blk['c2'][0], blk['stride'], blk['c3'][0], nxt['c1'][0], ds) and (
diff --git a/include/agrl_hip.h b/include/agrl_hip.h
--- a/include/agrl_hip.h
+++ b/include/agrl_hip.h
@@ -100,6 +100,10 @@
 int agrl_bottleneck_seam(const void* y2, const void* packed, const float* b3, const void* residual, void* out,
                          const float* b1_next, void* z, int M, int Cmid, int Cout, int Cnext, agrl_stream_t stream);
 
+int agrl_bottleneck_chain_enabled(int frames);
+int agrl_bottleneck_chain(const void* z1, const void* a0, const void* table, void* const* a_out, void* z_out, int frames, int n,
+                          agrl_stream_t stream);
+
 long long agrl_conv3x3_packed_bytes(int Cin, int Cout);
 int agrl_conv3x3_pack(const void* w_ohwi, void* packed, int Cin, int Cout, agrl_stream_t stream);
 int agrl_conv3x3_packed_bn_act(const void* x, const void* packed, const float* bias, void* out, int N, int H, int W, int Cin,
```

Result: faster. 76810 frames/s, median of 6 (+1.7%).
